# jedbrown/spectral-petsc

Measured on AMD Instinct MI355X. Metric: spectral matvecs/s and GB/s vs HBM roofline, 3D P^3 grid, higher is better.
Workload: dtype f64; 1 GPU; 3-D Poisson MatMult_Elliptic -dim 256,256,256 (gamma=0), global N(0,1) input seed 20240229; P=256, parallelism=single

## Files before the change

include/chebhip.h:

```cpp
#ifndef CHEBHIP_H
#define CHEBHIP_H

#ifdef __cplusplus
extern "C" {
#endif

enum {
  CHEBHIP_OK = 0,
  CHEBHIP_ERR_SIZE = 1,
  CHEBHIP_ERR_TDIM = 2,
  CHEBHIP_ERR_DIMS = 3,
  CHEBHIP_ERR_ARG = 4,
  CHEBHIP_ERR_DEVICE = 5,
  CHEBHIP_ERR_MEMORY = 6
};

const char *chebhip_last_error(void);
int chebhip_version(void);
const char *chebhip_arch(void);

typedef int (*chebhip_apply_fn)(void *ctx, const double *x_dev, double *y_dev, void *stream);
typedef int (*chebhip_reduce_fn)(void *ctx, double *vals_dev, int count, void *stream);

typedef struct cheb_plan cheb_plan;
// ... 41 lines not shown
int  cheb_modal_weights_host(int n, double *w);
int  cheb_modal_filter_matrix_host(int n, const double *sigma, double *F);

typedef struct cheb_points cheb_points;

int  cheb_points_create(int d, const int *dims, int nfields, cheb_points **out);
int  cheb_points_destroy(cheb_points *h);
long cheb_points_chunk(const cheb_points *h);
int  cheb_points_rows(cheb_points *h, int k, const double *x_dev, long m, double *R_dev, void *stream);
int  cheb_points_eval(cheb_points *h, const double *u_dev, const double *xi_dev, long npts, double *out_dev, void *stream);
enum { CHEB_SPREAD_ACCUMULATE = 1, CHEB_SPREAD_DELTA = 2 };
int  cheb_points_spread(cheb_points *h, const double *s_dev, const double *xi_dev, long npts, double *out_dev, int flags, void *stream);
long cheb_points_spread_pass(const cheb_points *h);
int  cheb_points_grid_reserve(cheb_points *h, const int *m_max);
int  cheb_points_eval_grid(cheb_points *h, const double *u_dev, const double *coords_dev, const int *m, double *out_dev, void *stream);
int  cheb_nodes_host(int n, double *x);
int  cheb_points_matrix_host(int n, int m, const double *x_host, double *R);
int  cheb_points_drows(cheb_points *h, int k, const double *x_dev, long m, double *R_dev, void *stream);
int  cheb_points_dmatrix_host(int n, int m, const double *x_host, double *R);
int  cheb_points_eval_deriv(cheb_points *h, const double *u_dev, const double *xi_dev, long npts, const int *deriv, double *out_dev,
                            void *stream);
int  cheb_points_spread_deriv(cheb_points *h, const double *s_dev, const double *xi_dev, long npts, const int *deriv, double *out_dev,
                              int flags, void *stream);
int  cheb_points_eval_grid_deriv(cheb_points *h, const double *u_dev, const double *coords_dev, const int *m, const int *deriv,
                                 double *out_dev, void *stream);
enum { CHEB_POINTS_GRAD_VALUE = 1 };
int  cheb_points_eval_grad(cheb_points *h, const double *u_dev, const double *xi_dev, long npts, const double *scale_host, int flags,
                           double *out_dev, void *stream);

typedef struct cheb_dealias cheb_dealias;

int  cheb_dealias_fine_size(int n);
int  cheb_dealias_matrix_host(int n, int m, int which, double *A);
int  cheb_dealias_create(int d, const int *dims, const int *dims_fine, int nfields, cheb_dealias **out);
int  cheb_dealias_destroy(cheb_dealias *h);
int  cheb_dealias_fine_dims(const cheb_dealias *h, int *dims_fine);
long cheb_dealias_size(const cheb_dealias *h);
long cheb_dealias_work_bytes(const cheb_dealias *h);
int  cheb_dealias_multiply(cheb_dealias *h, const double *u_dev, const double *v_dev, double *out_dev, void *stream);
int  cheb_dealias_reserve_advect(cheb_dealias *h);
int  cheb_dealias_advect(cheb_dealias *h, const double *vel_dev, const double *c_dev, double *out_dev, void *stream);

typedef struct cheb_reduce cheb_reduce;
enum { CHEB_W_INTEGRAL = 0, CHEB_W_MEAN = 1, CHEB_W_NODE = 2, CHEB_W_DNODE = 3, CHEB_W_POINT = 4, CHEB_W_DPOINT = 5 };

int  cheb_reduce_weights_host(int n, int kind, double arg, double *w);
int  cheb_reduce_create(int d, const int *dims, int nfields, const int *contract, cheb_reduce **out);
int  cheb_reduce_destroy(cheb_reduce *h);
int  cheb_reduce_set_weights(cheb_reduce *h, int k, const double *w_host);
long cheb_reduce_size(const cheb_reduce *h, int which);
int  cheb_reduce_slices(const cheb_reduce *h);
int  cheb_reduce_apply(cheb_reduce *h, const double *u_dev, const double *v_dev, double *out_dev, void *stream);

typedef struct cheb_stats cheb_stats;
enum { CHEB_STATS_UNIFORM = 0, CHEB_STATS_EDGES = 1 };

int  cheb_stats_spacing_host(int n, double *h);
int  cheb_stats_rate_host(int n, double s, double *r);
int  cheb_stats_check(int d, const int *dims, int nfields, int max_bins, int nbins);
int  cheb_stats_create(int d, const int *dims, int nfields, int max_bins, cheb_stats **out);
int  cheb_stats_destroy(cheb_stats *h);
int  cheb_stats_set_weights(cheb_stats *h, int k, const double *w_host);
long cheb_stats_size(const cheb_stats *h, int which);
int  cheb_stats_summary(cheb_stats *h, const double *u_dev, const double *center_dev, double *out_dev, void *stream);
int  cheb_stats_histogram(cheb_stats *h, const double *u_dev, const double *cond_dev, int mode, int nbins, const double *spec_dev,
                          double *out_dev, void *stream);
int  cheb_stats_cfl(cheb_stats *h, const double *vel_dev, const double *scale_host, double *out_dev, void *stream);

typedef struct cheb_grad cheb_grad;
enum { CHEB_INV_DIV = 1, CHEB_INV_VORT2 = 2, CHEB_INV_STRAIN2 = 4, CHEB_INV_GAMMA = 8, CHEB_INV_Q = 16, CHEB_INV_NORM2 = 32 };

int  cheb_grad_create(int d, const int *dims, const double *scale, cheb_grad **out);
int  cheb_grad_destroy(cheb_grad *h);
long cheb_grad_size(const cheb_grad *h);
long cheb_grad_work_size(const cheb_grad *h, int nfields);
int  cheb_grad_grad(cheb_grad *h, int nfields, const double *s_dev, double *out_dev, void *stream);
int  cheb_grad_tensor(cheb_grad *h, int nvec, const double *u_dev, double *G_dev, void *stream);
int  cheb_grad_div(cheb_grad *h, int nvec, const double *u_dev, double *out_dev, void *stream);
int  cheb_grad_curl(cheb_grad *h, int nvec, const double *u_dev, double *out_dev, void *stream);
int  cheb_grad_strain(cheb_grad *h, int nvec, const double *u_dev, double *out_dev, void *stream);
int  cheb_grad_laplacian(cheb_grad *h, int nfields, const double *s_dev, double *work_dev, double *out_dev, void *stream);
int  cheb_grad_invariants(cheb_grad *h, int nvec, const double *G_dev, unsigned mask, double *out_dev, void *stream);

typedef struct cheb_layout cheb_layout;
int  cheb_layout_create(int d, const int *dims, cheb_layout **out);
int  cheb_layout_destroy(cheb_layout *h);
long cheb_layout_size(const cheb_layout *h, int which);
int  cheb_layout_map_host(int d, const int *dims, int *map);
int  cheb_layout_unpack(cheb_layout *h, int ncomp, const double *xi_dev, long si, long oi, const double *xb_dev, long sb, long ob,
                        double *out_dev, void *stream);
int  cheb_layout_pack(cheb_layout *h, int ncomp, const double *fields_dev, double *xi_dev, long si, long oi, double *xb_dev, long sb, long ob,
                      void *stream);

typedef struct ell_op ell_op;

int ell_op_create(int d, const int *dims, ell_op **out);
int ell_op_destroy(ell_op *op);

long ell_op_local_size(const ell_op *op);
long ell_op_global_size(const ell_op *op);
long ell_op_dirichlet_size(const ell_op *op);

int ell_op_mult(ell_op *op, const double *U_dev, double *V_dev, void *stream);
int ell_op_mult_host(ell_op *op, const double *U_host, double *V_host);

int ell_op_function(ell_op *op, double gamma, double exponent, const double *U_dev,
                    const double *b_dev, double *rhs_dev, void *stream);
int ell_op_function_host(ell_op *op, double gamma, double exponent, const double *U_host,
                         const double *b_host, double *rhs_host);

int ell_op_set_dirichlet(ell_op *op, const double *values_host);

int ell_op_get_state(ell_op *op, int which, double *dst_host);
int ell_op_set_state(ell_op *op, int which, const double *src_host);

typedef int (*ell_dim0_fn)(void *ctx, int kind, int nfields, const double *in_dev, const double *acc_dev,
                           double alpha, double *out_dev, void *stream);
int ell_op_create_slab(int d, const int *dims, int lo, int hi, ell_dim0_fn dim0, void *dim0_ctx, ell_op **out);
int ell_op_pencil_sweep(ell_op *op, long ncol, const double *in_dev, double *out_dev, void *stream);

typedef struct stokes_op stokes_op;

int stokes_op_create(int d, const int *dims, stokes_op **out);
int stokes_op_destroy(stokes_op *op);
long stokes_op_size(const stokes_op *op, int which);

int stokes_op_set_rheology(stokes_op *op, int kind, double hardness, double exponent,
                           double regularization, double gamma0);
int stokes_op_set_dirichlet(stokes_op *op, const double *values_host);
int stokes_op_set_force(stokes_op *op, const double *force_host);

int stokes_op_mult(stokes_op *op, const double *xG_dev, double *yG_dev, void *stream);
int stokes_op_mult_vv(stokes_op *op, const double *vG_dev, double *vG_out_dev, void *stream);
int stokes_op_mult_pv(stokes_op *op, const double *vG_dev, double *pG_out_dev, void *stream);
int stokes_op_mult_vp(stokes_op *op, const double *pG_dev, double *vG_out_dev, void *stream);
int stokes_op_mult_schur(stokes_op *op, const double *pG_dev, double *pG_out_dev,
                         chebhip_apply_fn inner_solve, void *inner_ctx, void *stream);
int stokes_op_mult_vv_cm(stokes_op *op, const double *v_cm_dev, double *v_cm_out_dev, void *stream);
int stokes_op_mult_pv_cm(stokes_op *op, const double *v_cm_dev, double *pG_out_dev, void *stream);
int stokes_op_mult_vp_cm(stokes_op *op, const double *pG_dev, double *v_cm_out_dev, void *stream);
int stokes_op_mult_schur_cm(stokes_op *op, const double *pG_dev, double *pG_out_dev,
                            chebhip_apply_fn inner_solve_cm, void *inner_ctx, void *stream);
int stokes_op_set_inner_solver(stokes_op *op, int restart, double rtol, double atol, int max_it);
int stokes_op_inner_iterations(const stokes_op *op);
int stokes_op_set_inner_reduce(stokes_op *op, chebhip_reduce_fn reduce, void *ctx);
int stokes_op_function(stokes_op *op, const double *xG_dev, double *yG_dev, void *stream);
int stokes_op_get_state(stokes_op *op, int which, double *dst_host);
int stokes_op_set_state(stokes_op *op, int which, const double *src_host);

typedef int (*stokes_dim0_fn)(void *ctx, int kind, int nfields, const double *in_dev, const double *acc_dev,
                              double alpha, double *out_dev, void *stream);
int stokes_op_create_slab(int d, const int *dims, int lo, int hi, stokes_dim0_fn dim0, void *dim0_ctx, stokes_op **out);
int stokes_op_pencil_sweep(stokes_op *op, int nfields, long ncol, const double *in_dev, double *out_dev, void *stream);
int stokes_op_pencil_pressure(stokes_op *op, long ncol, double *p_pencil_dev, double *gp0_pencil_dev, void *stream);
int stokes_op_pencil_sweep_pressure(stokes_op *op, int nvel, long ncol, double *in_dev, double *out_dev, void *stream);

typedef struct chebhip_dist chebhip_dist;
typedef int (*chebhip_exchange_fn)(void *ctx, const double *send_dev, const long *send_counts, double *recv_dev,
                                   const long *recv_counts, void *stream);
int chebhip_dist_create(int d, const int *dims, int nranks, int rank, chebhip_dist **out);
int chebhip_dist_destroy(chebhip_dist *D);
long chebhip_dist_local_size(const chebhip_dist *D);
long chebhip_dist_slab_offset(const chebhip_dist *D);
int chebhip_dist_use_rccl(chebhip_dist *D, void *nccl_comm);
int chebhip_dist_set_exchange(chebhip_dist *D, chebhip_exchange_fn fn, void *ctx);
int chebhip_dist_mult(chebhip_dist *D, const double *U_slab_dev, double *V_slab_dev, void *stream);
int chebhip_dist_mult_batch(chebhip_dist *D, int nrhs, const double *U_slabs_dev, double *V_slabs_dev, void *stream);
int chebhip_rccl_unique_id(void *id128);
int chebhip_rccl_comm_create(int nranks, int rank, const void *id128, void **nccl_comm_out);
int chebhip_rccl_comm_destroy(void *nccl_comm);
int chebhip_rccl_reduce(void *nccl_comm, double *vals_dev, int count, void *stream);

typedef struct chebhip_comm chebhip_comm;
typedef struct chebhip_local_group chebhip_local_group;
typedef struct chebhip_ipc_group chebhip_ipc_group;
typedef int (*chebhip_exchangev_fn)(void *ctx, int nseg, const int *peers, const double *const *send_dev, const long *send_counts,
                                    double *const *recv_dev, const long *recv_counts, void *stream);
int chebhip_comm_create_rccl(void *nccl_comm, int nranks, int rank, chebhip_comm **out);
int chebhip_local_group_create(int nranks, chebhip_local_group **out);
int chebhip_local_group_destroy(chebhip_local_group *g);
int chebhip_local_group_abort(chebhip_local_group *g);
int chebhip_comm_create_local(chebhip_local_group *g, int rank, chebhip_comm **out);
int chebhip_comm_create_callback(int nranks, int rank, chebhip_exchangev_fn xfn, chebhip_reduce_fn rfn, void *ctx, chebhip_comm **out);
int chebhip_comm_create_null(int nranks, int rank, chebhip_comm **out);
int chebhip_comm_null_set_shadow(chebhip_comm *c, int k, const double *const *arrays);
int chebhip_ipc_group_open(const char *name, int nranks, int rank, chebhip_ipc_group **out);
int chebhip_ipc_group_close(chebhip_ipc_group *g);
int chebhip_ipc_group_abort(chebhip_ipc_group *g);
int chebhip_comm_create_ipc(chebhip_ipc_group *g, chebhip_comm *inner, chebhip_comm **out);
int chebhip_comm_destroy(chebhip_comm *c);
int chebhip_comm_size(const chebhip_comm *c);
int chebhip_comm_rank(const chebhip_comm *c);
int chebhip_comm_reduce(void *comm, double *vals_dev, int count, void *stream);
int chebhip_dist_use_comm(chebhip_dist *D, chebhip_comm *comm);

typedef struct chebhip_dist_stokes chebhip_dist_stokes;
typedef struct chebhip_fdpc chebhip_fdpc;
int chebhip_dist_stokes_create(int d, const int *dims, chebhip_comm *comm, chebhip_dist_stokes **out);
int chebhip_dist_stokes_destroy(chebhip_dist_stokes *D);
stokes_op *chebhip_dist_stokes_op(chebhip_dist_stokes *D);
int chebhip_dist_stokes_pc(chebhip_dist_stokes *D, chebhip_fdpc **out);
int chebhip_dist_stokes_ranges(const chebhip_dist_stokes *D, long *ranges4);
typedef struct chebhip_dist_ell chebhip_dist_ell;
int chebhip_dist_ell_create(int d, const int *dims, chebhip_comm *comm, chebhip_dist_ell **out);
int chebhip_dist_ell_destroy(chebhip_dist_ell *D);
ell_op *chebhip_dist_ell_op(chebhip_dist_ell *D);
int chebhip_dist_ell_pc(chebhip_dist_ell *D, chebhip_fdpc **out);
int chebhip_dist_ell_ranges(const chebhip_dist_ell *D, long *ranges4);

typedef struct chebhip_fgmres chebhip_fgmres;
int chebhip_fgmres_create(long n, int restart, chebhip_fgmres **out);
int chebhip_fgmres_set_reduce(chebhip_fgmres *k, chebhip_reduce_fn reduce, void *ctx);
int chebhip_fgmres_destroy(chebhip_fgmres *k);
int chebhip_fgmres_set_tolerances(chebhip_fgmres *k, double rtol, double atol, int max_it);
int chebhip_fgmres_solve(chebhip_fgmres *k, chebhip_apply_fn A, void *actx, chebhip_apply_fn M, void *mctx,
                         const double *b_dev, double *x_dev, int x_nonzero, void *stream);
int chebhip_fgmres_iterations(const chebhip_fgmres *k);
double chebhip_fgmres_residual(const chebhip_fgmres *k);
int chebhip_fgmres_reason(const chebhip_fgmres *k);

int ell_pc_create(ell_op *op, chebhip_fdpc **out);
int stokes_pc_create(stokes_op *op, chebhip_fdpc **out);
int chebhip_fdpc_destroy(chebhip_fdpc *pc);
typedef int (*chebhip_fdpc_dim0_fn)(void *ctx, int backward, int nfields, const double *in_dev, double *out_dev, void *stream);
int stokes_pc_create_slab(stokes_op *slab_op, long i0_offset, chebhip_fdpc_dim0_fn dim0, void *ctx, chebhip_fdpc **out);
int ell_pc_create_slab(ell_op *slab_op, long i0_offset, chebhip_fdpc_dim0_fn dim0, void *ctx, chebhip_fdpc **out);
int chebhip_fdpc_pencil_transform(chebhip_fdpc *pc, int backward, int nfields, long ncol, const double *in_dev, double *out_dev, void *stream);
int chebhip_fdpc_update(chebhip_fdpc *pc, void *stream);
int chebhip_fdpc_set_sweeps(chebhip_fdpc *pc, int sweeps);
int chebhip_fdpc_mult(chebhip_fdpc *pc, const double *x_dev, double *y_dev, void *stream);
int chebhip_fdpc_apply(void *pc, const double *r_dev, double *z_dev, void *stream);
int chebhip_fdpc_apply_cm(void *pc, const double *r_cm_dev, double *z_cm_dev, void *stream);
enum { CHEBHIP_FDPC_STEP_FORWARD = 0, CHEBHIP_FDPC_STEP_FORWARD_OVER_ETA = 1, CHEBHIP_FDPC_STEP_FORWARD_SCALED = 2,
       CHEBHIP_FDPC_STEP_ZSOLVE = 3, CHEBHIP_FDPC_STEP_SCALE = 4, CHEBHIP_FDPC_STEP_BACKWARD = 5 };
int chebhip_fdpc_step(chebhip_fdpc *pc, int k, int mode, const double *x_dev, double *y_dev, void *stream);
enum { CHEBHIP_FDPC_ROUTE_RAW = 1, CHEBHIP_FDPC_ROUTE_TWO_LAUNCH = 2, CHEBHIP_FDPC_ROUTE_GENERAL = 4, CHEBHIP_FDPC_ROUTE_FUSED_MUL = 8,
       CHEBHIP_FDPC_ROUTE_ETA_PASS = 16, CHEBHIP_FDPC_ROUTE_ZSOLVE = 32, CHEBHIP_FDPC_ROUTE_SCALE3 = 64, CHEBHIP_FDPC_ROUTE_SCALE_GENERAL = 128,
       CHEBHIP_FDPC_ROUTE_DENSE = 256 };
int chebhip_fdpc_step_route(chebhip_fdpc *pc, int k, int mode);
int chebhip_fdpc_line_host(int P, double *S, double *Sinv, double *lam);
int ell_pc_create_spectral(ell_op *op, double sigma, chebhip_fdpc **out);

typedef struct cheb_helmholtz cheb_helmholtz;
int  cheb_helmholtz_create(int d, const int *dims, double sigma, int nfields, cheb_helmholtz **out);
int  cheb_helmholtz_solve(cheb_helmholtz *h, const double *f_dev, double *u_dev, void *stream);
int  cheb_helmholtz_apply(void *h, const double *x_dev, double *y_dev, void *stream);
int  cheb_helmholtz_destroy(cheb_helmholtz *h);
long cheb_helmholtz_size(const cheb_helmholtz *h);
int  cheb_helmholtz_line_host(int P, double *S, double *Sinv, double *lam);
chebhip_fdpc *cheb_helmholtz_fdpc(cheb_helmholtz *h);

int  cheb_helmholtz_create_bc(int d, const int *dims, const double *bc, double sigma, int nfields, cheb_helmholtz **out);
int  cheb_helmholtz_solve_bc(cheb_helmholtz *h, const double *f_dev, const double *g_dev, double *u_dev, void *stream);
long cheb_helmholtz_full_size(const cheb_helmholtz *h);
long cheb_helmholtz_boundary_size(const cheb_helmholtz *h);
int  cheb_helmholtz_singular(const cheb_helmholtz *h);
int  cheb_helmholtz_line_bc_host(int P, const double *bc4, double *S, double *Sinv, double *lam,
                                 double *Q , double *L , double *Binv );
int  cheb_helmholtz_create_box(int d, const int *dims, const double *bc, const double *scale, double sigma, int nfields, cheb_helmholtz **out);
int  cheb_helmholtz_line_box_host(int P, const double *bc4, double s, double *S, double *Sinv, double *lam,
                                  double *Q , double *L , double *Binv );

typedef struct cheb_project cheb_project;
enum { CHEB_FACE_WALL = 0, CHEB_FACE_OPEN = 1 };
int  cheb_project_create(int d, const int *dims, const int *faces, const double *scale, int nvec, cheb_project **out);
int  cheb_project_destroy(cheb_project *h);
long cheb_project_size(const cheb_project *h, int which);
int  cheb_project_singular(const cheb_project *h);
int  cheb_project_faces_host(int d, const int *dims, int *face);
int  cheb_project_apply(cheb_project *h, const double *u_dev, const double *flux_dev, double *phi_dev, double *out_dev, void *stream);

typedef struct cheb_opfun cheb_opfun;
enum { CHEB_OPFUN_ONE = 0, CHEB_OPFUN_INV, CHEB_OPFUN_RES, CHEB_OPFUN_EXP, CHEB_OPFUN_PHI1, CHEB_OPFUN_PHI2, CHEB_OPFUN_PHI3, CHEB_OPFUN_POW };
typedef struct { int out, in, kind; double coef, tau, par; } cheb_opfun_term;
int  cheb_opfun_create(int d, const int *dims, const double *bc, const double *scale, double sigma, int nin, int nout, cheb_opfun **out);
int  cheb_opfun_destroy(cheb_opfun *h);
int  cheb_opfun_set_terms(cheb_opfun *h, int nterms, const cheb_opfun_term *terms);
int  cheb_opfun_check_terms(int nin, int nout, int nterms, const cheb_opfun_term *terms);
int  cheb_opfun_apply(cheb_opfun *h, const double *x_dev, double *y_dev, void *stream);
int  cheb_opfun_apply_full(cheb_opfun *h, const double *x_dev, double *yfull_dev, void *stream);
long cheb_opfun_size(const cheb_opfun *h, int which);
int  cheb_opfun_singular(const cheb_opfun *h);
int  cheb_opfun_weight_host(int kind, double tau, double par, double s, double *w);
int  cheb_opfun_weights_host(int kind, double tau, double par, long n, const double *s, double *w);
int  cheb_opfun_eval(int kind, double tau, double par, const double *s_dev, long n, double *w_dev, void *stream);

typedef struct stokes_saddle stokes_saddle;
int stokes_saddle_create(stokes_op *op, stokes_saddle **out);
int stokes_saddle_create_slab(stokes_op *slab_op, chebhip_fdpc *slab_pc, chebhip_reduce_fn reduce, void *reduce_ctx, stokes_saddle **out);
int stokes_saddle_destroy(stokes_saddle *s);
int stokes_saddle_set_type(stokes_saddle *s, int type);
int stokes_saddle_set_inner(stokes_saddle *s, int which, int max_it, double rtol);
int stokes_saddle_set_schur_jacobi(stokes_saddle *s, int on);
int stokes_saddle_set_pc_sweeps(stokes_saddle *s, int sweeps);
int stokes_saddle_setup(stokes_saddle *s, void *stream);
int stokes_saddle_apply(void *s, const double *x_dev, double *y_dev, void *stream);
int stokes_saddle_iterations(const stokes_saddle *s, int which);

int chebhip_set_option(const char *name, int value);
int chebhip_get_option(const char *name, int *value);
const char *chebhip_option_name(int index);

long chebhip_launch_count(void);

enum {
  CHEBHIP_STAGE_CHEB_APPLY = 0, CHEBHIP_STAGE_ELL_MULT, CHEBHIP_STAGE_ELL_FUNCTION, CHEBHIP_STAGE_STOKES_MULT,
  CHEBHIP_STAGE_STOKES_MULT_VV, CHEBHIP_STAGE_STOKES_MULT_PV, CHEBHIP_STAGE_STOKES_MULT_VP, CHEBHIP_STAGE_STOKES_FUNCTION,
  CHEBHIP_STAGE_STOKES_SCHUR, CHEBHIP_STAGE_FDPC_APPLY, CHEBHIP_STAGE_SADDLE_APPLY, CHEBHIP_STAGE_FGMRES_SOLVE,
  CHEBHIP_NSTAGES
};
int chebhip_timers_enable(int on);
int chebhip_timers_reset(void);
int chebhip_timers_read(int stage, double *total_ms, long *calls);
const char *chebhip_stage_name(int stage);

int stokes_op_viscosity_range(stokes_op *op, double *eta_min, double *eta_max, void *stream);
int stokes_op_write_vtk(stokes_op *op, const double *state_dev, const char *path);

#ifdef __cplusplus
}
#endif
#endif
```

spectral-petsc_amd/__init__.py:

```python
import ctypes as C
import os
import subprocess

_HERE = os.path.dirname(os.path.abspath(__file__))
LIB_PATH = os.environ.get("CHEBHIP_LIB_PATH") or os.path.join(_HERE, "libchebhip.so")
INCLUDE_DIR = os.path.join(os.path.dirname(_HERE), "include")

ABI_SYMBOLS = [
    "chebhip_last_error", "chebhip_version", "chebhip_arch", "chebhip_launch_count",
    "chebhip_set_option", "chebhip_get_option", "chebhip_option_name",
    "cheb_plan_create", "cheb_apply", "cheb_apply_host", "cheb_plan_destroy", "cheb_plan_size",
    "cheb_plan_create_trimmed", "cheb_apply_lap1d", "cheb_slab_pack", "cheb_slab_unpack_add",
    "ell_op_create", "ell_op_destroy", "ell_op_local_size", "ell_op_global_size",
    "ell_op_dirichlet_size", "ell_op_mult", "ell_op_mult_host", "ell_op_function",
    "ell_op_function_host", "ell_op_set_dirichlet", "ell_op_get_state", "ell_op_set_state",
    "ell_op_create_slab", "ell_op_pencil_sweep",
    "stokes_op_create", "stokes_op_destroy", "stokes_op_size", "stokes_op_set_rheology",
    "stokes_op_set_dirichlet", "stokes_op_set_force", "stokes_op_mult", "stokes_op_mult_vv",
    "stokes_op_mult_pv", "stokes_op_mult_vp", "stokes_op_mult_vv_cm", "stokes_op_mult_pv_cm", "stokes_op_mult_vp_cm", "stokes_op_mult_schur_cm", "stokes_op_function", "stokes_op_get_state",
    "stokes_op_set_state", "stokes_op_create_slab", "stokes_op_pencil_sweep", "stokes_op_pencil_pressure", "stokes_op_pencil_sweep_pressure", "stokes_op_mult_schur", "stokes_op_set_inner_solver", "stokes_op_inner_iterations", "stokes_op_set_inner_reduce",
    "chebhip_fgmres_create", "chebhip_fgmres_destroy", "chebhip_fgmres_set_tolerances", "chebhip_fgmres_solve",
    "chebhip_fgmres_iterations", "chebhip_fgmres_residual", "chebhip_fgmres_reason", "chebhip_fgmres_set_reduce",
    "ell_pc_create", "stokes_pc_create", "chebhip_fdpc_destroy", "chebhip_fdpc_update", "chebhip_fdpc_set_sweeps",
    "chebhip_fdpc_mult", "chebhip_fdpc_apply", "chebhip_fdpc_apply_cm",
    "chebhip_fdpc_step", "chebhip_fdpc_step_route", "chebhip_fdpc_line_host", "cheb_helmholtz_fdpc",
    "stokes_saddle_create", "stokes_saddle_destroy", "stokes_saddle_set_type", "stokes_saddle_set_inner",
    "stokes_saddle_setup", "stokes_saddle_apply", "stokes_saddle_iterations", "stokes_saddle_set_pc_sweeps", "stokes_saddle_set_schur_jacobi",
    "chebhip_timers_enable", "chebhip_timers_reset", "chebhip_timers_read", "chebhip_stage_name",
    "stokes_op_viscosity_range", "stokes_op_write_vtk",
    "chebhip_dist_create", "chebhip_dist_destroy", "chebhip_dist_local_size", "chebhip_dist_slab_offset",
    "chebhip_dist_use_rccl", "chebhip_dist_set_exchange", "chebhip_dist_mult", "chebhip_dist_mult_batch",
    "chebhip_rccl_unique_id", "chebhip_rccl_comm_create", "chebhip_rccl_comm_destroy", "chebhip_rccl_reduce",
    "chebhip_comm_create_rccl", "chebhip_local_group_create", "chebhip_local_group_destroy", "chebhip_local_group_abort",
    "chebhip_comm_create_local", "chebhip_comm_create_callback", "chebhip_comm_create_null", "chebhip_comm_null_set_shadow", "chebhip_comm_destroy", "chebhip_comm_size", "chebhip_comm_rank",
    "chebhip_ipc_group_open", "chebhip_ipc_group_close", "chebhip_ipc_group_abort", "chebhip_comm_create_ipc",
    "chebhip_comm_reduce", "chebhip_dist_use_comm",
    "chebhip_dist_stokes_create", "chebhip_dist_stokes_destroy", "chebhip_dist_stokes_op", "chebhip_dist_stokes_ranges",
    "chebhip_dist_ell_create", "chebhip_dist_ell_destroy", "chebhip_dist_ell_op", "chebhip_dist_ell_ranges",
    "stokes_pc_create_slab", "ell_pc_create_slab", "chebhip_fdpc_pencil_transform", "chebhip_dist_stokes_pc", "chebhip_dist_ell_pc",
    "stokes_saddle_create_slab",
    "cheb_resample_create", "cheb_resample_apply", "cheb_resample_destroy", "cheb_resample_size", "cheb_resample_matrix_host",
    "cheb_helmholtz_create", "cheb_helmholtz_solve", "cheb_helmholtz_apply", "cheb_helmholtz_destroy", "cheb_helmholtz_size",
    "cheb_helmholtz_line_host", "ell_pc_create_spectral",
    "cheb_helmholtz_create_bc", "cheb_helmholtz_solve_bc", "cheb_helmholtz_full_size", "cheb_helmholtz_boundary_size",
    "cheb_helmholtz_singular", "cheb_helmholtz_line_bc_host",
    "cheb_modal_create", "cheb_modal_destroy", "cheb_modal_size", "cheb_modal_spectrum_size", "cheb_modal_forward", "cheb_modal_backward",
    "cheb_modal_set_filter", "cheb_modal_filter", "cheb_modal_spectrum", "cheb_modal_integrate",
    "cheb_modal_matrix_host", "cheb_modal_weights_host", "cheb_modal_filter_matrix_host",
    "cheb_points_create", "cheb_points_destroy", "cheb_points_chunk", "cheb_points_rows", "cheb_points_eval",
    "cheb_points_spread", "cheb_points_spread_pass",
    "cheb_points_grid_reserve", "cheb_points_eval_grid", "cheb_nodes_host", "cheb_points_matrix_host",
    "cheb_points_drows", "cheb_points_dmatrix_host", "cheb_points_eval_deriv", "cheb_points_spread_deriv",
    "cheb_points_eval_grid_deriv", "cheb_points_eval_grad",
    "cheb_dealias_fine_size", "cheb_dealias_matrix_host", "cheb_dealias_create", "cheb_dealias_destroy", "cheb_dealias_fine_dims",
    "cheb_dealias_size", "cheb_dealias_work_bytes", "cheb_dealias_multiply", "cheb_dealias_reserve_advect", "cheb_dealias_advect",
    "cheb_reduce_weights_host", "cheb_reduce_create", "cheb_reduce_destroy", "cheb_reduce_set_weights", "cheb_reduce_size",
    "cheb_reduce_slices", "cheb_reduce_apply",
    "cheb_stats_spacing_host", "cheb_stats_rate_host", "cheb_stats_check", "cheb_stats_create", "cheb_stats_destroy",
    "cheb_stats_set_weights", "cheb_stats_size", "cheb_stats_summary", "cheb_stats_histogram", "cheb_stats_cfl",
    "cheb_grad_create", "cheb_grad_destroy", "cheb_grad_size", "cheb_grad_work_size", "cheb_grad_grad", "cheb_grad_tensor",
    "cheb_grad_div", "cheb_grad_curl", "cheb_grad_strain", "cheb_grad_laplacian", "cheb_grad_invariants",
    "cheb_layout_create", "cheb_layout_destroy", "cheb_layout_size", "cheb_layout_map_host", "cheb_layout_unpack", "cheb_layout_pack",
    "cheb_helmholtz_create_box", "cheb_helmholtz_line_box_host",
    "cheb_project_create", "cheb_project_destroy", "cheb_project_size", "cheb_project_singular", "cheb_project_faces_host",
    "cheb_project_apply",
    "cheb_opfun_create", "cheb_opfun_destroy", "cheb_opfun_set_terms", "cheb_opfun_apply", "cheb_opfun_apply_full", "cheb_opfun_size",
    "cheb_opfun_singular", "cheb_opfun_check_terms", "cheb_opfun_weight_host", "cheb_opfun_weights_host", "cheb_opfun_eval",
]


class OpFunTerm(C.Structure):
    _fields_ = [("out", C.c_int), ("inp", C.c_int), ("kind", C.c_int), ("coef", C.c_double), ("tau", C.c_double), ("par", C.c_double)]


class ChebhipError(RuntimeError):
    def __init__(self, code, msg):
        super().__init__("chebhip error %d: %s" % (code, msg))
        self.code = code


def build(force=False):
    src = os.path.join(_HERE, "csrc")
    if force:
        subprocess.check_call(["make", "-C", src, "-s", "clean"])
    subprocess.check_call(["make", "-C", src, "-s"])
    return LIB_PATH


_lib = None


def lib():
    global _lib
    if _lib is None:
        if not os.path.exists(LIB_PATH):
            raise ChebhipError(-1, "libchebhip.so not built (run __graft_entry__.build()); there is no CPU fallback")
        L = C.CDLL(LIB_PATH)
        dp, ip, vp = C.POINTER(C.c_double), C.POINTER(C.c_int), C.c_void_p
        L.chebhip_last_error.restype = C.c_char_p
        L.chebhip_arch.restype = C.c_char_p
        L.chebhip_launch_count.restype = C.c_long
        L.chebhip_set_option.argtypes = [C.c_char_p, C.c_int]
        L.chebhip_get_option.argtypes = [C.c_char_p, C.POINTER(C.c_int)]
        L.chebhip_option_name.argtypes = [C.c_int]
        L.chebhip_option_name.restype = C.c_char_p
        L.cheb_plan_create.argtypes = [C.c_int, C.c_int, ip, C.POINTER(vp)]
        L.cheb_apply.argtypes = [vp, vp, vp, vp]
        L.cheb_plan_create_trimmed.argtypes = [C.c_int, C.c_int, ip, C.POINTER(vp)]
        L.cheb_apply_lap1d.argtypes = [vp, vp, vp, C.c_double, vp, vp]
        lp = C.POINTER(C.c_long)
        L.cheb_slab_pack.argtypes = [C.c_long, C.c_long, C.c_long, C.c_int, lp, vp, vp, vp]
        L.cheb_slab_unpack_add.argtypes = [C.c_long, C.c_long, C.c_long, C.c_int, lp, vp, vp, C.c_double, vp, vp]
        L.cheb_apply_host.argtypes = [vp, dp, dp]
        L.cheb_plan_destroy.argtypes = [vp]
        L.cheb_plan_size.argtypes = [vp]
        L.cheb_plan_size.restype = C.c_long
        L.ell_op_create.argtypes = [C.c_int, ip, C.POINTER(vp)]
        L.ell_op_destroy.argtypes = [vp]
        L.ell_op_create_slab.argtypes = [C.c_int, ip, C.c_int, C.c_int, vp, vp, C.POINTER(vp)]
        L.ell_op_pencil_sweep.argtypes = [vp, C.c_long, vp, vp, vp]
        for f in (L.ell_op_local_size, L.ell_op_global_size, L.ell_op_dirichlet_size):
            f.argtypes = [vp]
            f.restype = C.c_long
        L.ell_op_mult.argtypes = [vp, vp, vp, vp]
        L.ell_op_mult_host.argtypes = [vp, dp, dp]
        L.ell_op_function.argtypes = [vp, C.c_double, C.c_double, vp, vp, vp, vp]
        L.ell_op_function_host.argtypes = [vp, C.c_double, C.c_double, dp, dp, dp]
        L.ell_op_set_dirichlet.argtypes = [vp, dp]
        L.ell_op_get_state.argtypes = [vp, C.c_int, dp]
        L.ell_op_set_state.argtypes = [vp, C.c_int, dp]
        L.stokes_op_create.argtypes = [C.c_int, ip, C.POINTER(vp)]
        L.stokes_op_destroy.argtypes = [vp]
        L.stokes_op_size.argtypes = [vp, C.c_int]
        L.stokes_op_size.restype = C.c_long
        L.stokes_op_set_rheology.argtypes = [vp, C.c_int, C.c_double, C.c_double, C.c_double, C.c_double]
        L.stokes_op_set_dirichlet.argtypes = [vp, dp]
        L.stokes_op_set_force.argtypes = [vp, dp]
        for f in (L.stokes_op_mult, L.stokes_op_mult_vv, L.stokes_op_mult_pv, L.stokes_op_mult_vp, L.stokes_op_function,
                  L.stokes_op_mult_vv_cm, L.stokes_op_mult_pv_cm, L.stokes_op_mult_vp_cm):
            f.argtypes = [vp, vp, vp, vp]
        L.stokes_op_mult_schur_cm.argtypes = [vp, vp, vp, vp, vp, vp]
        L.stokes_op_get_state.argtypes = [vp, C.c_int, dp]
        L.stokes_op_set_state.argtypes = [vp, C.c_int, dp]
        L.stokes_op_create_slab.argtypes = [C.c_int, ip, C.c_int, C.c_int, vp, vp, C.POINTER(vp)]
        L.stokes_op_pencil_sweep.argtypes = [vp, C.c_int, C.c_long, vp, vp, vp]
        L.stokes_op_pencil_pressure.argtypes = [vp, C.c_long, vp, vp, vp]
        L.stokes_op_mult_schur.argtypes = [vp, vp, vp, vp, vp, vp]
        L.stokes_op_set_inner_solver.argtypes = [vp, C.c_int, C.c_double, C.c_double, C.c_int]
        L.stokes_op_inner_iterations.argtypes = [vp]
        L.stokes_op_set_inner_reduce.argtypes = [vp, vp, vp]
        L.chebhip_fgmres_create.argtypes = [C.c_long, C.c_int, C.POINTER(vp)]
        L.chebhip_fgmres_destroy.argtypes = [vp]
        L.chebhip_fgmres_set_tolerances.argtypes = [vp, C.c_double, C.c_double, C.c_int]
        L.chebhip_fgmres_solve.argtypes = [vp, vp, vp, vp, vp, vp, vp, C.c_int, vp]
        L.chebhip_fgmres_iterations.argtypes = [vp]
        L.chebhip_fgmres_residual.argtypes = [vp]
        L.chebhip_fgmres_residual.restype = C.c_double
        L.chebhip_fgmres_reason.argtypes = [vp]
        L.chebhip_fgmres_set_reduce.argtypes = [vp, vp, vp]
        L.ell_pc_create.argtypes = [vp, C.POINTER(vp)]
        L.stokes_pc_create.argtypes = [vp, C.POINTER(vp)]
        L.chebhip_fdpc_destroy.argtypes = [vp]
        L.chebhip_fdpc_update.argtypes = [vp, vp]
        L.chebhip_fdpc_set_sweeps.argtypes = [vp, C.c_int]
        L.chebhip_fdpc_mult.argtypes = [vp, vp, vp, vp]
        L.chebhip_fdpc_apply.argtypes = [vp, vp, vp, vp]
        L.chebhip_fdpc_apply_cm.argtypes = [vp, vp, vp, vp]
        L.stokes_saddle_create.argtypes = [vp, C.POINTER(vp)]
        L.stokes_saddle_destroy.argtypes = [vp]
        L.stokes_saddle_set_type.argtypes = [vp, C.c_int]
        L.stokes_saddle_set_inner.argtypes = [vp, C.c_int, C.c_int, C.c_double]
        L.stokes_saddle_setup.argtypes = [vp, vp]
        L.stokes_saddle_apply.argtypes = [vp, vp, vp, vp]
        L.stokes_saddle_iterations.argtypes = [vp, C.c_int]
        L.stokes_saddle_set_pc_sweeps.argtypes = [vp, C.c_int]
        L.stokes_saddle_set_schur_jacobi.argtypes = [vp, C.c_int]
        L.chebhip_timers_enable.argtypes = [C.c_int]
        L.chebhip_timers_read.argtypes = [C.c_int, dp, C.POINTER(C.c_long)]
        L.chebhip_stage_name.argtypes = [C.c_int]
        L.chebhip_stage_name.restype = C.c_char_p
        L.stokes_op_viscosity_range.argtypes = [vp, dp, dp, vp]
        L.stokes_op_write_vtk.argtypes = [vp, vp, C.c_char_p]
        L.chebhip_dist_create.argtypes = [C.c_int, ip, C.c_int, C.c_int, C.POINTER(vp)]
        L.chebhip_dist_destroy.argtypes = [vp]
        for f in (L.chebhip_dist_local_size, L.chebhip_dist_slab_offset):
            f.argtypes = [vp]
            f.restype = C.c_long
        L.chebhip_dist_use_rccl.argtypes = [vp, vp]
        L.chebhip_dist_set_exchange.argtypes = [vp, vp, vp]
        L.chebhip_dist_mult.argtypes = [vp, vp, vp, vp]
        L.chebhip_dist_mult_batch.argtypes = [vp, C.c_int, vp, vp, vp]
        L.chebhip_rccl_unique_id.argtypes = [vp]
        L.chebhip_rccl_comm_create.argtypes = [C.c_int, C.c_int, vp, C.POINTER(vp)]
        L.chebhip_rccl_comm_destroy.argtypes = [vp]
        L.chebhip_rccl_reduce.argtypes = [vp, vp, C.c_int, vp]
        L.chebhip_comm_create_rccl.argtypes = [vp, C.c_int, C.c_int, C.POINTER(vp)]
        L.chebhip_local_group_create.argtypes = [C.c_int, C.POINTER(vp)]
        L.chebhip_local_group_destroy.argtypes = [vp]
        L.chebhip_local_group_abort.argtypes = [vp]
        L.chebhip_comm_create_local.argtypes = [vp, C.c_int, C.POINTER(vp)]
        L.chebhip_comm_create_callback.argtypes = [C.c_int, C.c_int, vp, vp, vp, C.POINTER(vp)]
        L.chebhip_comm_destroy.argtypes = [vp]
        L.chebhip_comm_create_null.argtypes = [C.c_int, C.c_int, C.POINTER(vp)]
        L.chebhip_comm_null_set_shadow.argtypes = [vp, C.c_int, C.POINTER(vp)]
        L.chebhip_ipc_group_open.argtypes = [C.c_char_p, C.c_int, C.c_int, C.POINTER(vp)]
        L.chebhip_ipc_group_close.argtypes = [vp]
        L.chebhip_ipc_group_abort.argtypes = [vp]
        L.chebhip_comm_create_ipc.argtypes = [vp, vp, C.POINTER(vp)]
        L.chebhip_comm_size.argtypes = [vp]
        L.chebhip_comm_rank.argtypes = [vp]
        L.chebhip_comm_reduce.argtypes = [vp, vp, C.c_int, vp]
        L.chebhip_dist_use_comm.argtypes = [vp, vp]
        for nm in ("stokes", "ell"):
            getattr(L, "chebhip_dist_%s_create" % nm).argtypes = [C.c_int, ip, vp, C.POINTER(vp)]
            getattr(L, "chebhip_dist_%s_destroy" % nm).argtypes = [vp]
            getattr(L, "chebhip_dist_%s_op" % nm).argtypes = [vp]
            getattr(L, "chebhip_dist_%s_op" % nm).restype = vp
            getattr(L, "chebhip_dist_%s_ranges" % nm).argtypes = [vp, lp]
            getattr(L, "chebhip_dist_%s_pc" % nm).argtypes = [vp, C.POINTER(vp)]
            getattr(L, "%s_pc_create_slab" % nm).argtypes = [vp, C.c_long, vp, vp, C.POINTER(vp)]
        L.chebhip_fdpc_pencil_transform.argtypes = [vp, C.c_int, C.c_int, C.c_long, vp, vp, vp]
        L.stokes_saddle_create_slab.argtypes = [vp, vp, vp, vp, C.POINTER(vp)]
        L.cheb_resample_create.argtypes = [C.c_int, ip, C.c_int, ip, C.c_int, C.c_int, C.POINTER(vp)]
        L.cheb_resample_apply.argtypes = [vp, vp, vp, vp]
        L.cheb_resample_destroy.argtypes = [vp]
        L.cheb_resample_size.argtypes = [vp, C.c_int]
        L.cheb_resample_size.restype = C.c_long
        L.cheb_resample_matrix_host.argtypes = [C.c_int, C.c_int, C.c_int, C.c_int, dp]
        L.cheb_helmholtz_create.argtypes = [C.c_int, ip, C.c_double, C.c_int, C.POINTER(vp)]
        for f in (L.cheb_helmholtz_solve, L.cheb_helmholtz_apply):
            f.argtypes = [vp, vp, vp, vp]
        L.cheb_helmholtz_destroy.argtypes = [vp]
        L.cheb_helmholtz_size.argtypes = [vp]
        L.cheb_helmholtz_size.restype = C.c_long
        L.cheb_helmholtz_line_host.argtypes = [C.c_int, dp, dp, dp]
        L.chebhip_fdpc_line_host.argtypes = [C.c_int, dp, dp, dp]
        L.chebhip_fdpc_step.argtypes = [vp, C.c_int, C.c_int, vp, vp, vp]
        L.chebhip_fdpc_step_route.argtypes = [vp, C.c_int, C.c_int]
        L.cheb_helmholtz_fdpc.argtypes = [vp]
        L.cheb_helmholtz_fdpc.restype = vp
        L.ell_pc_create_spectral.argtypes = [vp, C.c_double, C.POINTER(vp)]
        L.cheb_helmholtz_create_bc.argtypes = [C.c_int, ip, dp, C.c_double, C.c_int, C.POINTER(vp)]
        L.cheb_helmholtz_solve_bc.argtypes = [vp, vp, vp, vp, vp]
        for f in (L.cheb_helmholtz_full_size, L.cheb_helmholtz_boundary_size):
            f.argtypes = [vp]
            f.restype = C.c_long
        L.cheb_helmholtz_singular.argtypes = [vp]
        L.cheb_helmholtz_line_bc_host.argtypes = [C.c_int, dp, dp, dp, dp, dp, dp, dp]
        L.cheb_modal_create.argtypes = [C.c_int, ip, C.c_int, C.POINTER(vp)]
        L.cheb_modal_destroy.argtypes = [vp]
        for f in (L.cheb_modal_size, L.cheb_modal_spectrum_size):
            f.argtypes = [vp]
            f.restype = C.c_long
        for f in (L.cheb_modal_forward, L.cheb_modal_backward, L.cheb_modal_filter, L.cheb_modal_spectrum):
            f.argtypes = [vp, vp, vp, vp]
        L.cheb_modal_set_filter.argtypes = [vp, C.c_int, dp]
        L.cheb_modal_integrate.argtypes = [vp, vp, vp, vp, vp]
        L.cheb_modal_matrix_host.argtypes = [C.c_int, C.c_int, dp]
        L.cheb_modal_weights_host.argtypes = [C.c_int, dp]
        L.cheb_modal_filter_matrix_host.argtypes = [C.c_int, dp, dp]
        L.cheb_points_create.argtypes = [C.c_int, ip, C.c_int, C.POINTER(vp)]
        L.cheb_points_destroy.argtypes = [vp]
        L.cheb_points_chunk.argtypes = [vp]
        L.cheb_points_chunk.restype = C.c_long
        L.cheb_points_rows.argtypes = [vp, C.c_int, vp, C.c_long, vp, vp]
        L.cheb_points_eval.argtypes = [vp, vp, vp, C.c_long, vp, vp]
        L.cheb_points_spread.argtypes = [vp, vp, vp, C.c_long, vp, C.c_int, vp]
        L.cheb_points_spread_pass.argtypes = [vp]
        L.cheb_points_spread_pass.restype = C.c_long
        L.cheb_points_grid_reserve.argtypes = [vp, ip]
        L.cheb_points_eval_grid.argtypes = [vp, vp, vp, ip, vp, vp]
        L.cheb_nodes_host.argtypes = [C.c_int, dp]
        L.cheb_points_matrix_host.argtypes = [C.c_int, C.c_int, dp, dp]
        L.cheb_points_drows.argtypes = [vp, C.c_int, vp, C.c_long, vp, vp]
        L.cheb_points_dmatrix_host.argtypes = [C.c_int, C.c_int, dp, dp]
        L.cheb_points_eval_deriv.argtypes = [vp, vp, vp, C.c_long, ip, vp, vp]
        L.cheb_points_spread_deriv.argtypes = [vp, vp, vp, C.c_long, ip, vp, C.c_int, vp]
        L.cheb_points_eval_grid_deriv.argtypes = [vp, vp, vp, ip, ip, vp, vp]
        L.cheb_points_eval_grad.argtypes = [vp, vp, vp, C.c_long, dp, C.c_int, vp, vp]
        L.cheb_dealias_fine_size.argtypes = [C.c_int]
        L.cheb_dealias_matrix_host.argtypes = [C.c_int, C.c_int, C.c_int, dp]
        L.cheb_dealias_create.argtypes = [C.c_int, ip, ip, C.c_int, C.POINTER(vp)]
        L.cheb_dealias_destroy.argtypes = [vp]
        L.cheb_dealias_fine_dims.argtypes = [vp, ip]
        for f in (L.cheb_dealias_size, L.cheb_dealias_work_bytes):
            f.argtypes = [vp]
            f.restype = C.c_long
        L.cheb_dealias_reserve_advect.argtypes = [vp]
        for f in (L.cheb_dealias_multiply, L.cheb_dealias_advect):
            f.argtypes = [vp, vp, vp, vp, vp]
        L.cheb_reduce_weights_host.argtypes = [C.c_int, C.c_int, C.c_double, dp]
        L.cheb_reduce_create.argtypes = [C.c_int, ip, C.c_int, ip, C.POINTER(vp)]
        L.cheb_reduce_destroy.argtypes = [vp]
        L.cheb_reduce_set_weights.argtypes = [vp, C.c_int, dp]
        L.cheb_reduce_size.argtypes = [vp, C.c_int]
        L.cheb_reduce_size.restype = C.c_long
        L.cheb_reduce_slices.argtypes = [vp]
        L.cheb_reduce_apply.argtypes = [vp, vp, vp, vp, vp]
        L.cheb_stats_spacing_host.argtypes = [C.c_int, dp]
        L.cheb_stats_rate_host.argtypes = [C.c_int, C.c_double, dp]
        L.cheb_stats_check.argtypes = [C.c_int, ip, C.c_int, C.c_int, C.c_int]
        L.cheb_stats_create.argtypes = [C.c_int, ip, C.c_int, C.c_int, C.POINTER(vp)]
        L.cheb_stats_destroy.argtypes = [vp]
        L.cheb_stats_set_weights.argtypes = [vp, C.c_int, dp]
        L.cheb_stats_size.argtypes = [vp, C.c_int]
        L.cheb_stats_size.restype = C.c_long
        L.cheb_stats_summary.argtypes = [vp, vp, vp, vp, vp]
        L.cheb_stats_histogram.argtypes = [vp, vp, vp, C.c_int, C.c_int, vp, vp, vp]
        L.cheb_stats_cfl.argtypes = [vp, vp, dp, vp, vp]
        L.cheb_grad_create.argtypes = [C.c_int, ip, dp, C.POINTER(vp)]
        L.cheb_grad_destroy.argtypes = [vp]
        L.cheb_grad_size.argtypes = [vp]
        L.cheb_grad_size.restype = C.c_long
        L.cheb_grad_work_size.argtypes = [vp, C.c_int]
        L.cheb_grad_work_size.restype = C.c_long
        for f in (L.cheb_grad_grad, L.cheb_grad_tensor, L.cheb_grad_div, L.cheb_grad_curl, L.cheb_grad_strain):
            f.argtypes = [vp, C.c_int, vp, vp, vp]
        L.cheb_grad_laplacian.argtypes = [vp, C.c_int, vp, vp, vp, vp]
        L.cheb_grad_invariants.argtypes = [vp, C.c_int, vp, C.c_uint, vp, vp]
        L.cheb_layout_create.argtypes = [C.c_int, ip, C.POINTER(vp)]
        L.cheb_layout_destroy.argtypes = [vp]
        L.cheb_layout_size.argtypes = [vp, C.c_int]
        L.cheb_layout_size.restype = C.c_long
        L.cheb_layout_map_host.argtypes = [C.c_int, ip, ip]
        L.cheb_layout_unpack.argtypes = [vp, C.c_int, vp, C.c_long, C.c_long, vp, C.c_long, C.c_long, vp, vp]
        L.cheb_layout_pack.argtypes = [vp, C.c_int, vp, vp, C.c_long, C.c_long, vp, C.c_long, C.c_long, vp]
        L.cheb_helmholtz_create_box.argtypes = [C.c_int, ip, dp, dp, C.c_double, C.c_int, C.POINTER(vp)]
        L.cheb_helmholtz_line_box_host.argtypes = [C.c_int, dp, C.c_double, dp, dp, dp, dp, dp, dp]
        L.cheb_project_create.argtypes = [C.c_int, ip, ip, dp, C.c_int, C.POINTER(vp)]
        L.cheb_project_destroy.argtypes = [vp]
        L.cheb_project_size.argtypes = [vp, C.c_int]
        L.cheb_project_size.restype = C.c_long
        L.cheb_project_singular.argtypes = [vp]
        L.cheb_project_faces_host.argtypes = [C.c_int, ip, ip]
        L.cheb_project_apply.argtypes = [vp, vp, vp, vp, vp, vp]
        L.cheb_opfun_create.argtypes = [C.c_int, ip, dp, dp, C.c_double, C.c_int, C.c_int, C.POINTER(vp)]
        L.cheb_opfun_destroy.argtypes = [vp]
        L.cheb_opfun_set_terms.argtypes = [vp, C.c_int, C.POINTER(OpFunTerm)]
        L.cheb_opfun_check_terms.argtypes = [C.c_int, C.c_int, C.c_int, C.POINTER(OpFunTerm)]
        L.cheb_opfun_apply.argtypes = [vp, vp, vp, vp]
        L.cheb_opfun_apply_full.argtypes = [vp, vp, vp, vp]
        L.cheb_opfun_size.argtypes = [vp, C.c_int]
        L.cheb_opfun_size.restype = C.c_long
        L.cheb_opfun_singular.argtypes = [vp]
        L.cheb_opfun_weight_host.argtypes = [C.c_int, C.c_double, C.c_double, C.c_double, dp]
        L.cheb_opfun_weights_host.argtypes = [C.c_int, C.c_double, C.c_double, C.c_long, dp, dp]
        L.cheb_opfun_eval.argtypes = [C.c_int, C.c_double, C.c_double, vp, C.c_long, vp, vp]
        _lib = L
    return _lib


def set_option(name, value):
    _chk(lib().chebhip_set_option(name.encode(), int(value)))


def get_option(name):
    v = C.c_int()
    _chk(lib().chebhip_get_option(name.encode(), C.byref(v)))
    return v.value


def options():
    out, i = {}, 0
    while True:
        n = lib().chebhip_option_name(i).decode()
        if not n:
            return out
        out[n] = get_option(n)
        i += 1


def _chk(rc):
    if rc != 0:
        raise ChebhipError(rc, lib().chebhip_last_error().decode())


def _ints(v):
    return (C.c_int * len(v))(*[int(x) for x in v])


def _np_dp(a):
    import numpy as np
    assert isinstance(a, np.ndarray) and a.dtype == np.float64 and a.flags["C_CONTIGUOUS"]
    return a.ctypes.data_as(C.POINTER(C.c_double))


def _dev_ptr(t, n):
    import torch
    assert isinstance(t, torch.Tensor) and t.is_cuda and t.dtype == torch.float64 and t.is_contiguous()
    assert t.numel() == n, "expected %d elements, got %d" % (n, t.numel())
    return t.data_ptr()


def _stream():
    import torch
    return torch.cuda.current_stream().cuda_stream


def device_view(ptr, n):
    import torch

    if not ptr or int(n) == 0:
        return torch.empty(0, dtype=torch.float64, device=torch.device("cuda", torch.cuda.current_device()))

# ... 1467 lines not shown
```

spectral-petsc_amd/csrc/chebhip.hip:

```cpp
#include "../../include/chebhip.h"
#include "sweep.h"
#include "ops.h"
#include "timers.h"
#include <atomic>
#include <mutex>
#include <cmath>
#include <cstdarg>
#include <cstdio>
#include <cstdlib>
#include <cstring>
#include <map>
#include <new>
#include <string>
#include <vector>

using namespace chebhip;

static thread_local std::string g_err;
int chebhip_fail(int code, const char *fmt, ...) {
  char buf[512];
  va_list ap; va_start(ap, fmt); vsnprintf(buf, sizeof buf, fmt, ap); va_end(ap);
  g_err = buf;
  return code;
}

extern "C" const char *chebhip_last_error(void) { return g_err.c_str(); }
extern "C" int chebhip_version(void) { return 100; }
extern "C" const char *chebhip_arch(void) { return "gfx950"; }
extern "C" long chebhip_launch_count(void) { return sweep_launch_count(); }

extern "C" int chebhip_set_option(const char *name, int value) {
  if (!name) return chebhip_fail(CHEBHIP_ERR_ARG, "NULL option name");
  if (!strcmp(name, "no_rocblas")) { opt_set(OPT_VENDOR_GEMM, value ? 0 : 1); return 0; }
  const int id = opt_find(name);
  if (id < 0) return chebhip_fail(CHEBHIP_ERR_ARG, "unknown option '%s'", name);
  opt_set(id, value);
  return 0;
}
extern "C" int chebhip_get_option(const char *name, int *value) {
  if (!name || !value) return chebhip_fail(CHEBHIP_ERR_ARG, "NULL argument");
  if (!strcmp(name, "no_rocblas")) { *value = opt(OPT_VENDOR_GEMM) ? 0 : 1; return 0; }
  const int id = opt_find(name);
  if (id < 0) return chebhip_fail(CHEBHIP_ERR_ARG, "unknown option '%s'", name);
  *value = opt(id);
  return 0;
}
extern "C" const char *chebhip_option_name(int index) { return opt_name(index); }
static const double *g_stamp_buf = nullptr;
static int g_stamp_cnt = 0;
extern "C" void chebhip_debug_stamp_buffer(const void *dev) { g_stamp_buf = (const double *)dev; g_stamp_cnt = 0; }
const double *chebhip_stamp_buf() { return g_stamp_buf; }
int chebhip_stamp_next() { return g_stamp_cnt++; }

namespace {
struct Pending { int id; hipEvent_t e0, e1; };
std::mutex g_tm_mu;
bool g_tm_on = false;
std::vector<Pending> g_tm_pending;
double g_tm_ms[CHEBHIP_NSTAGES] = {0};
long g_tm_calls[CHEBHIP_NSTAGES] = {0};
const char *const g_tm_names[CHEBHIP_NSTAGES] = {
  "cheb_apply", "ell_op_mult", "ell_op_function", "stokes_op_mult", "stokes_op_mult_vv", "stokes_op_mult_pv", "stokes_op_mult_vp",
  "stokes_op_function", "stokes_op_mult_schur", "chebhip_fdpc_apply", "stokes_saddle_apply", "chebhip_fgmres_solve"};
void tm_drain_locked() {
  for (auto &p : g_tm_pending) {
    float ms = 0.f;
    if (hipEventSynchronize(p.e1) == hipSuccess && hipEventElapsedTime(&ms, p.e0, p.e1) == hipSuccess) { g_tm_ms[p.id] += ms; g_tm_calls[p.id]++; }
    (void)hipEventDestroy(p.e0); (void)hipEventDestroy(p.e1);
  }
  g_tm_pending.clear();
}
}
chebhip::StageTimer::StageTimer(int stage, void *stream) : id(stage), st((hipStream_t)stream), on(g_tm_on) {
  if (!on) return;
  if (hipEventCreate(&e0) != hipSuccess || hipEventRecord(e0, st) != hipSuccess) { on = false; if (e0) (void)hipEventDestroy(e0); }
}
chebhip::StageTimer::~StageTimer() {
  if (!on) return;
  hipEvent_t e1 = nullptr;
  if (hipEventCreate(&e1) != hipSuccess || hipEventRecord(e1, st) != hipSuccess) { (void)hipEventDestroy(e0); if (e1) (void)hipEventDestroy(e1); return; }
  std::lock_guard<std::mutex> lk(g_tm_mu);
  g_tm_pending.push_back({id, e0, e1});
  if (g_tm_pending.size() > 4096) tm_drain_locked();
}
extern "C" int chebhip_timers_enable(int on) { std::lock_guard<std::mutex> lk(g_tm_mu); g_tm_on = on != 0; return 0; }
extern "C" int chebhip_timers_reset(void) {
  std::lock_guard<std::mutex> lk(g_tm_mu);
  tm_drain_locked();
  for (int i = 0; i < CHEBHIP_NSTAGES; i++) { g_tm_ms[i] = 0.0; g_tm_calls[i] = 0; }
  return 0;
}
extern "C" int chebhip_timers_read(int stage, double *total_ms, long *calls) {
  if (stage < 0 || stage >= CHEBHIP_NSTAGES || !total_ms || !calls) return chebhip_fail(CHEBHIP_ERR_ARG, "stage %d out of range", stage);
  std::lock_guard<std::mutex> lk(g_tm_mu);
  tm_drain_locked();
  *total_ms = g_tm_ms[stage]; *calls = g_tm_calls[stage];
  return 0;
}
extern "C" const char *chebhip_stage_name(int stage) { return (stage >= 0 && stage < CHEBHIP_NSTAGES) ? g_tm_names[stage] : ""; }

struct cheb_plan {
  int rank = 0, tr = 0;
  std::vector<int> dims;
  long N = 0;
  unsigned inner = 1, ncols = 0;
  DiffMat mat;
  DiffMat lap;
  bool trimmed = false;
  double *hx = nullptr, *hy = nullptr;
};

static int check_geom(int rank, int tr, const int *dims, long *N, unsigned *inner, bool allow_long = false) {
  if (!dims || rank < 1 || rank > 16) return chebhip_fail(CHEBHIP_ERR_DIMS, "rank = %d must be in 1..16", rank);
  if (!(0 <= tr && tr < rank)) return chebhip_fail(CHEBHIP_ERR_TDIM, "tdim out of range");
  long n = 1, in = 1;
  for (int r = 0; r < rank; r++) {
    if (dims[r] < 1) return chebhip_fail(CHEBHIP_ERR_DIMS, "dims[%d] = %d must be >= 1", r, dims[r]);
    n *= dims[r];
    if (r > tr) in *= dims[r];
    if (n > 0x7fffffffL) return chebhip_fail(CHEBHIP_ERR_DIMS, "tensor of more than 2^31-1 points");
  }
  if (n < 2 || dims[tr] < 2) return chebhip_fail(CHEBHIP_ERR_SIZE, "n = %ld but must be >= 2", n);
  if (dims[tr] > 256 && !allow_long)
    return chebhip_fail(CHEBHIP_ERR_ARG, "dims[tr] = %d: the interior-layout (slab) plans support <= 256 points per line", dims[tr]);
  if (dims[tr] > 4096) return chebhip_fail(CHEBHIP_ERR_ARG, "dims[tr] = %d: at most 4096 points per line", dims[tr]);
  *N = n; *inner = (unsigned)in;
  return 0;
}

extern "C" int cheb_plan_create(int rank, int tr, const int *dims, cheb_plan **out) {
  if (!out) return chebhip_fail(CHEBHIP_ERR_ARG, "out is NULL");
  *out = nullptr;
  long N; unsigned inner;
  int rc = check_geom(rank, tr, dims, &N, &inner, true);
  if (rc) return rc;
  if ((rc = require_device())) return rc;
  cheb_plan *p = new (std::nothrow) cheb_plan;
  if (!p) return chebhip_fail(CHEBHIP_ERR_MEMORY, "out of host memory");
  p->rank = rank; p->tr = tr; p->dims.assign(dims, dims + rank);
  p->N = N; p->inner = inner; p->ncols = (unsigned)(N / dims[tr]);
  hipError_t e = hipSuccess;
  e = diffmat_create(dims[tr], &p->mat);
  if (e != hipSuccess) { delete p; return chebhip_fail(CHEBHIP_ERR_DEVICE, "plan matrices: %s", hipGetErrorString(e)); }
  *out = p;
  return 0;
}

extern "C" long cheb_plan_size(const cheb_plan *p) { return p ? p->N : -1; }

extern "C" int cheb_plan_create_trimmed(int rank, int tr, const int *dims, cheb_plan **out) {
  if (!out) return chebhip_fail(CHEBHIP_ERR_ARG, "out is NULL");
  *out = nullptr;
  if (!dims || rank < 1 || rank > 16) return chebhip_fail(CHEBHIP_ERR_DIMS, "rank = %d must be in 1..16", rank);
  if (!(0 <= tr && tr < rank)) return chebhip_fail(CHEBHIP_ERR_TDIM, "tdim out of range");
  std::vector<int> full(dims, dims + rank);
  if (dims[tr] < 1) return chebhip_fail(CHEBHIP_ERR_SIZE, "dims[tr] = %d stored points but must be >= 1", dims[tr]);
  full[tr] = dims[tr] + 2;
  long N; unsigned inner;
  int rc = check_geom(rank, tr, full.data(), &N, &inner);
  if (rc) return rc;
  if ((rc = require_device())) return rc;
  cheb_plan *p = new (std::nothrow) cheb_plan;
  if (!p) return chebhip_fail(CHEBHIP_ERR_MEMORY, "out of host memory");
  p->rank = rank; p->tr = tr; p->dims.assign(dims, dims + rank); p->trimmed = true;
  p->N = N / full[tr] * dims[tr]; p->inner = inner; p->ncols = (unsigned)(N / full[tr]);
  hipError_t e = diffmat_create(full[tr], &p->mat);
  if (e == hipSuccess) e = diffmat_create_lap(full[tr], &p->lap);
  if (e != hipSuccess) { diffmat_destroy(&p->mat); delete p; return chebhip_fail(CHEBHIP_ERR_DEVICE, "diffmat_create: %s", hipGetErrorString(e)); }
  *out = p;
  return 0;
}

extern "C" int cheb_apply_lap1d(cheb_plan *p, const double *x, const double *acc, double alpha,
                                double *y, void *stream) {
  if (!p || !x || !y) return chebhip_fail(CHEBHIP_ERR_ARG, "NULL argument");
  if (!p->trimmed) return chebhip_fail(CHEBHIP_ERR_ARG, "cheb_apply_lap1d needs a plan from cheb_plan_create_trimmed");
  if (x == y) return chebhip_fail(CHEBHIP_ERR_ARG, "x and y must be distinct");
  SweepParams sp = {};
  sp.ncols = p->ncols; sp.inner = p->inner;
  sp.in0 = x; sp.in_mode = IN_PLAIN;
  sp.alpha = alpha; sp.out = y;
  if (acc) { sp.out_mode = OUT_ACC; sp.acc = acc; } else sp.out_mode = OUT_STORE;
  HIP_TRY(sweep_launch(p->lap, sp, (hipStream_t)stream));
  return 0;
}

namespace chebhip {
int lap1d_gather_try(cheb_plan *p, const GatherSrc &g, double alpha, double *y, hipStream_t st, bool *done) {
  *done = false;
  if (!p || !p->trimmed || !y) return 0;
  SweepParams sp = {};
  sp.ncols = p->ncols; sp.inner = p->inner;
  sp.in_mode = IN_PLAIN; sp.alpha = alpha; sp.out = y; sp.out_mode = OUT_STORE;
  HIP_TRY(sweep_launch_gather(p->lap, sp, g, st, done));
  return 0;
}
}

namespace chebhip {
int lap1d_multi_gather_try(int n, cheb_plan *const *plans, const double *x, double *const *outs, cheb_plan *gp, const GatherSrc &g, double *gout,
                           double alpha, hipStream_t st, bool *done) {
  *done = false;
  if (n < 1 || n > 8 || !gp || !gp->trimmed || !gout) return 0;
  const DiffMat *m[9]; SweepParams sp[9];
  for (int k = 0; k < n; k++) {
    if (!plans[k] || !plans[k]->trimmed) return 0;
    sp[k] = SweepParams{};
    sp[k].ncols = plans[k]->ncols; sp[k].inner = plans[k]->inner;
    sp[k].in0 = x; sp[k].in_mode = IN_PLAIN; sp[k].alpha = alpha; sp[k].out = outs[k]; sp[k].out_mode = OUT_STORE;
    m[k] = &plans[k]->lap;
  }
  sp[n] = SweepParams{};
  sp[n].ncols = gp->ncols; sp[n].inner = gp->inner; sp[n].in_mode = IN_PLAIN; sp[n].alpha = alpha; sp[n].out = gout; sp[n].out_mode = OUT_STORE;
  m[n] = &gp->lap;
  HIP_TRY(sweep_launch_multi_gather_try(n + 1, m, sp, 1u << n, g, st, done));
  return 0;
}
}

namespace chebhip {
int lap1d_multi_try(int n, cheb_plan *const *plans, const double *x, double *const *outs, double alpha, hipStream_t st, bool *done) {
  *done = false;
  if (n < 2 || n > 9) return 0;
  const DiffMat *m[9]; SweepParams sp[9];
  for (int k = 0; k < n; k++) {
    if (!plans[k] || !plans[k]->trimmed) return 0;
    sp[k] = SweepParams{};
    sp[k].ncols = plans[k]->ncols; sp[k].inner = plans[k]->inner;
    sp[k].in0 = x; sp[k].in_mode = IN_PLAIN; sp[k].alpha = alpha; sp[k].out = outs[k]; sp[k].out_mode = OUT_STORE;
    m[k] = &plans[k]->lap;
  }
  HIP_TRY(sweep_launch_multi_try(n, m, sp, st, done));
  return 0;
}
}

extern "C" int cheb_apply(cheb_plan *p, const double *x, double *y, void *stream) {
  if (!p || !x || !y) return chebhip_fail(CHEBHIP_ERR_ARG, "NULL argument");
  if (x == y) return chebhip_fail(CHEBHIP_ERR_ARG, "x and y must be distinct (as every ChebMult call site)");
  if (p->trimmed) return chebhip_fail(CHEBHIP_ERR_ARG, "plan is trimmed: use cheb_apply_lap1d");
  StageTimer tm(CHEBHIP_STAGE_CHEB_APPLY, stream);
  SweepParams sp = {};
  sp.ncols = p->ncols; sp.inner = p->inner;
  sp.in0 = x; sp.out = y; sp.alpha = 1.0;
  sp.in_mode = IN_PLAIN; sp.out_mode = OUT_STORE;
  HIP_TRY(sweep_launch(p->mat, sp, (hipStream_t)stream));
  return 0;
}

extern "C" int cheb_apply_host(cheb_plan *p, const double *x, double *y) {
  if (!p || !x || !y) return chebhip_fail(CHEBHIP_ERR_ARG, "NULL argument");
  const size_t bytes = (size_t)p->N * sizeof(double);
  if (!p->hx) { HIP_TRY(hipMalloc((void **)&p->hx, bytes)); HIP_TRY(hipMalloc((void **)&p->hy, bytes)); }
  HIP_TRY(hipMemcpy(p->hx, x, bytes, hipMemcpyHostToDevice));
  int rc = cheb_apply(p, p->hx, p->hy, nullptr);
  if (rc) return rc;
  HIP_TRY(hipMemcpy(y, p->hy, bytes, hipMemcpyDeviceToHost));
  return 0;
}

extern "C" int cheb_plan_destroy(cheb_plan *p) {
  if (!p) return 0;
  diffmat_destroy(&p->mat);
  diffmat_destroy(&p->lap);
  if (p->hx) (void)hipFree(p->hx);
  if (p->hy) (void)hipFree(p->hy);
  delete p;
  return 0;
}

struct SlabSplit { int G; long c1[65]; };

__device__ __forceinline__ long slab_buf_index(const SlabSplit &sp, long m0, long M1, long R, long e) {
  const long i0 = e / (M1 * R), rem = e - i0 * (M1 * R);
  const long j = rem / R, r = rem - j * R;
  int s = 0;
  while (s + 1 < sp.G && j >= sp.c1[s + 1]) s++;
  const long w = sp.c1[s + 1] - sp.c1[s];
  return m0 * sp.c1[s] * R + (i0 * w + (j - sp.c1[s])) * R + r;
}

__global__ void k_slab_pack(SlabSplit sp, long m0, long M1, long R, const double *__restrict__ slab, double *__restrict__ buf) {
  const long n = m0 * M1 * R;
  for (long e = blockIdx.x * (long)blockDim.x + threadIdx.x; e < n; e += (long)gridDim.x * blockDim.x)
    buf[slab_buf_index(sp, m0, M1, R, e)] = slab[e];
}

__global__ void k_slab_unpack_add(SlabSplit sp, long m0, long M1, long R, const double *__restrict__ buf,
                                  const double *acc, double alpha, double *out) {
  const long n = m0 * M1 * R;
  for (long e = blockIdx.x * (long)blockDim.x + threadIdx.x; e < n; e += (long)gridDim.x * blockDim.x) {
    const double t = alpha * buf[slab_buf_index(sp, m0, M1, R, e)];
    out[e] = acc ? acc[e] + t : t;
  }
}

static int slab_split(int G, const long *c1, long M1, SlabSplit *sp) {
  if (G < 1 || G > 64 || !c1) return chebhip_fail(CHEBHIP_ERR_ARG, "G = %d must be in 1..64", G);
  sp->G = G;
  for (int s = 0; s <= G; s++) {
    sp->c1[s] = c1[s];
    if (c1[s] < 0 || c1[s] > M1 || (s > 0 && c1[s] < c1[s - 1])) return chebhip_fail(CHEBHIP_ERR_ARG, "column splits must be non-decreasing in 0..M1");
  }
  if (c1[0] != 0 || c1[G] != M1) return chebhip_fail(CHEBHIP_ERR_ARG, "column splits must cover 0..M1");
  return 0;
}

extern "C" int cheb_slab_pack(long m0, long M1, long R, int G, const long *c1, const double *slab, double *buf, void *stream) {
  if (!slab || !buf || m0 < 0 || M1 < 0 || R < 1) return chebhip_fail(CHEBHIP_ERR_ARG, "bad argument");
  SlabSplit sp; int rc = slab_split(G, c1, M1, &sp); if (rc) return rc;
  const long n = m0 * M1 * R;
  if (n == 0) return 0;
  long g = (n + 255) / 256; if (g > 4096) g = 4096;
  hipLaunchKernelGGL(k_slab_pack, dim3((unsigned)g), dim3(256), 0, (hipStream_t)stream, sp, m0, M1, R, slab, buf);
  HIP_TRY(hipGetLastError());
  return 0;
}

extern "C" int cheb_slab_unpack_add(long m0, long M1, long R, int G, const long *c1, const double *buf, const double *acc,
                                    double alpha, double *out, void *stream) {
  if (!buf || !out || m0 < 0 || M1 < 0 || R < 1) return chebhip_fail(CHEBHIP_ERR_ARG, "bad argument");
  SlabSplit sp; int rc = slab_split(G, c1, M1, &sp); if (rc) return rc;
  const long n = m0 * M1 * R;
  if (n == 0) return 0;
  long g = (n + 255) / 256; if (g > 4096) g = 4096;
  hipLaunchKernelGGL(k_slab_unpack_add, dim3((unsigned)g), dim3(256), 0, (hipStream_t)stream, sp, m0, M1, R, buf, acc, alpha, out);
  HIP_TRY(hipGetLastError());
  return 0;
}

__global__ void k_gather_bc(long N, const int *__restrict__ ixL, const double *__restrict__ U,
                            const double *__restrict__ dirloc, double *__restrict__ w0) {
// ... 808 lines not shown
```

spectral-petsc_amd/csrc/sweep.h:

```cpp
#pragma once
#include <hip/hip_runtime.h>
#include <vector>

namespace chebhip {

enum InMode : int {
  IN_PLAIN = 0,
  IN_GATHER = 1,
  IN_FLUX_ETA = 2,
  IN_FLUX_FULL = 3,
  IN_SUM3 = 4,
  IN_MUL = 5
};

enum OutMode : int {
  OUT_STORE = 0,
  OUT_ACC = 1,
  OUT_ACC_SCATTER = 2,
  OUT_ACC2 = 4,
  OUT_MUL = 3
};

enum CoefMode : int {
  COEF_UNIT = 0,
  COEF_ETA = 1,
  COEF_FULL = 2
};

struct SweepParams {
  int P;
  int H;
  unsigned ncols;
  unsigned inner;
  const double *in0, *in1, *in2, *in3, *in4;
  double *out;
  const double *acc;
  const double *acc2;
  const int *gcol;
  long gstride;
  double alpha;
  int in_mode, out_mode;
  const double *fragE, *fragO;
  const double *fragE2, *fragO2;
  const double *longDT;
  const double *longD;
  const double *zero;
  double *sink;
  unsigned ntiles;
  int sym;
  int raw;
  int trim;
  int coef_mode;
  double *gout;
  unsigned nouter, qmax;
  unsigned in_os, in_rs, acc_os, acc_rs, out_os, out_rs;
  unsigned in_bytes, acc_bytes, out_bytes;
  unsigned in_fblocks, in_fskip;
  unsigned in_fblocks_inv;
  unsigned gfield0;
};

struct DiffMat {
  int P = 0, H = 0;
  int KS = 0;
  int MTP = 0;
  double *fragE = nullptr, *fragO = nullptr;
  double *fragE2 = nullptr, *fragO2 = nullptr;
  double *longDT = nullptr;
  double *longD = nullptr;
  double *zero = nullptr;
  double *sink = nullptr;
  int sym = 0;
  int xl_ks = 0;
};

hipError_t diffmat_create(int P, DiffMat *out);
hipError_t diffmat_create_lap(int P, DiffMat *out);
hipError_t diffmat_create_pext(int P, DiffMat *out);
hipError_t diffmat_create_dd(int P, DiffMat *out);
void diffmat_destroy(DiffMat *m);
hipError_t diffmat_from_dense(int M, const long double *A, int sym, DiffMat *out);
hipError_t diffmat_from_blocks(int M, const long double *ME, const long double *MO, int sym, DiffMat *out);
void diffmat_dense_host(int P, double *D);
void resample_matrix_host(int n_in, int in_interior, int n_out, int out_interior, double *R);
void modal_matrix_host(int n, int which, double *M);
void modal_weights_host(int n, double *w);
void modal_filter_matrix_host(int n, const double *sigma, double *F);
int dealias_fine_size(int n);
void dealias_matrix_host(int n, int m, int which, double *A);
void points_nodes_host(int n, double *x);
void points_matrix_host(int n, int m, const double *x, double *R);
void points_dmatrix_host(int n, int m, const double *x, double *R);
enum { REDUCE_W_INTEGRAL = 0, REDUCE_W_MEAN, REDUCE_W_NODE, REDUCE_W_DNODE, REDUCE_W_POINT, REDUCE_W_DPOINT };
int reduce_weights_host(int n, int kind, double arg, double *w);
void stats_spacing_host(int n, double *h);
void stats_rate_host(int n, double s, double *r);

hipError_t sweep_launch(const DiffMat &m, SweepParams p, hipStream_t stream);

hipError_t fused_launch(const DiffMat &m, SweepParams p, hipStream_t stream);
void sweep_note_launch();

struct ResampleDir {
  const double *R;
  const double *x;
  double *y;
  unsigned O, K, M, Q, L;
};
hipError_t resample_launch(const ResampleDir &p, hipStream_t stream);
struct LineStep { int dir; const double *R; int m; };
hipError_t line_chain(int d, long *cur, long outer, long inner, int nsteps, const LineStep *steps, const double *src, double *dst,
                      double *const *work, hipStream_t stream);

struct F4Geom { unsigned os, ls, rs; };
struct Fused4Params {
  int P, H;
  unsigned nouter, qmax, ntiles, tpo, tpo_inv;
  const double *in; F4Geom gi; unsigned in_bytes;
  const void *coef; F4Geom gc; unsigned coef_bytes;
  double *gout; unsigned gout_bytes;
  const double *acc; F4Geom ga; unsigned acc_bytes;
  double *out; F4Geom go; unsigned out_bytes;
  const double *sub; unsigned sub_bytes;
  int trimf;
  double *w0out; unsigned w0_bytes;
  double alpha;
  int eta_square; double gamma4;
  const double *fragE2, *fragO2;
};
bool fused4_eligible(const DiffMat &m);
hipError_t fused4_launch(const DiffMat &m, Fused4Params p, bool jfast, bool full, bool acc, bool win, hipStream_t stream);

bool sweep_xl_eligible(const DiffMat &m, const SweepParams &p);
hipError_t sweep_xl_launch(const DiffMat &m, SweepParams p, hipStream_t stream);

bool sweep_vec_eligible(const DiffMat &m, const SweepParams &p);
bool sweep_takes_vec(const DiffMat &m, const SweepParams &p);
bool sweep_vec_raw_eligible(const DiffMat &m, const SweepParams &p);
hipError_t sweep_vec_launch(const DiffMat &m, SweepParams p, hipStream_t stream);
constexpr int GATHER_MAX = 16;
struct GatherSrc { const double *p[GATHER_MAX]; int s0[GATHER_MAX + 1]; unsigned lq[GATHER_MAX]; int pmax[GATHER_MAX]; int G; unsigned rowlen, col0;
                   double *dp[GATHER_MAX]; int push; };
hipError_t sweep_launch_gather(const DiffMat &m, SweepParams p, const GatherSrc &g, hipStream_t stream, bool *done);
hipError_t sweep_vec_launch_gather(const DiffMat &m, SweepParams p, const GatherSrc &g, hipStream_t stream, bool *done);
hipError_t sweep_vec_launch_multi(int n, const DiffMat *const *m, SweepParams *jobs, hipStream_t stream, bool *done);
hipError_t sweep_vec_launch_multi_gather(int n, const DiffMat *const *m, SweepParams *jobs, unsigned gmask, const GatherSrc &g, hipStream_t stream, bool *done);
hipError_t sweep_launch_multi_gather_try(int n, const DiffMat *const *m, const SweepParams *p, unsigned gmask, const GatherSrc &g, hipStream_t stream, bool *done);
hipError_t sweep_launch_multi(int n, const DiffMat *const *m, const SweepParams *p, hipStream_t stream);
hipError_t sweep_launch_multi_try(int n, const DiffMat *const *m, const SweepParams *p, hipStream_t stream, bool *done);

long sweep_launch_count();
}
struct cheb_plan;
struct stokes_op;
struct ell_op;
namespace chebhip {
bool ell_pencil_gather_supported(const ell_op *op);
int ell_pencil_gather_try(ell_op *op, long ncol, const GatherSrc &g, double *out, hipStream_t st, bool *done);
int stokes_pencil_gather_try(stokes_op *op, int kind, int nf, long ncol, const GatherSrc &g, double *out, hipStream_t st, bool *done);
bool stokes_pencil_gather_supported(const stokes_op *op);
int lap1d_multi_try(int n, cheb_plan *const *plans, const double *x, double *const *outs, double alpha, hipStream_t st, bool *done);
int lap1d_gather_try(cheb_plan *p, const GatherSrc &g, double alpha, double *y, hipStream_t st, bool *done);
int lap1d_multi_gather_try(int n, cheb_plan *const *plans, const double *x, double *const *outs, cheb_plan *gp, const GatherSrc &g, double *gout,
                           double alpha, hipStream_t st, bool *done);
int sweep_num_cus(hipError_t *err);

enum OptId { OPT_GENERAL_KERNELS = 0, OPT_SEPARATE_LAUNCHES, OPT_VENDOR_GEMM, OPT_NO_RAW_TRANSFORMS, OPT_EQUAL_SHARES, OPT_FORCE_GEMM,
             OPT_STOKES_SINGLE_STREAM, OPT_ETA_FROM_MEMORY, OPT_GATHER_PASS, OPT_RCCL_SELF_MESSAGES, OPT_LOCAL_TIMEOUT_S, OPT_FULL_STRESS, OPT_DIST_SINGLE_STREAM, OPT_LONG_LINES_GEMM, OPT_PRESSURE_PASSES, OPT_GENERAL_VISCOUS, OPT_POISSON_LAUNCHES, OPT_DIST_EXACT_ORDER, OPT_FDM_PASSES, OPT_SADDLE_NODE_MAJOR, OPT_STOKES_Z_SEPARATE, OPT_FDM_Z_SEPARATE, OPT_STOKES_PRESSURE_STREAM, OPT_KRYLOV_EXACT_NORM, OPT_STOKES_PRESSURE_SWEEPS, OPT_DIST_PACKED_EXCHANGE, OPT_POINTS_SPREAD_PASS, OPT_SWEEP_ALPHA_MULTIPLY, OPT_COUNT };
int opt(int id);
void opt_set(int id, int value);
const char *opt_name(int id);
int opt_find(const char *name);

bool fdm_line(int P, std::vector<long double> &S, std::vector<long double> &Sinv, std::vector<long double> &lam);
bool spec_line(int P, std::vector<long double> &S, std::vector<long double> &Sinv, std::vector<long double> &lam);
enum { SPEC_BC_SIZE = 1, SPEC_BC_COND, SPEC_BC_SINGULAR, SPEC_BC_EIG };
int spec_line_bc(int P, const double *bc4, std::vector<long double> &S, std::vector<long double> &Sinv, std::vector<long double> &lam,
                 std::vector<long double> &Q, std::vector<long double> &L, std::vector<long double> &Binv, bool &parity);
void centro_part(int M, const std::vector<long double> &A, int part, std::vector<long double> &out);

}
```

spectral-petsc_amd/csrc/sweep_vec.hip:

```cpp
#include "sweep.h"
#include "tile.h"
#include <cstdlib>
#include <type_traits>

const double *chebhip_stamp_buf();
int chebhip_stamp_next();

namespace chebhip {

template <bool ALIGNED16>
__device__ __forceinline__ void lds_put2(double *dst, double __attribute__((ext_vector_type(2))) v) {
  if (ALIGNED16) *(double __attribute__((ext_vector_type(2))) *)dst = v;
  else { dst[0] = v.x; dst[1] = v.y; }
}

template <int KS, bool JFAST, bool SUM3 = false, bool ACC = true>
__device__ __forceinline__ void vec1_body(const SweepParams &p, double *smem, const u32 BID, const u32 NBLK) {
  static_assert(KS <= 8, "lines of more than 64 points run vec4_body");
  static_assert(!SUM3 || !ACC, "IN_SUM3 exists for plain stores only");
  using G = TileGeom<KS, JFAST>;
  static_assert(G::CH >= 1 && (G::QSTEP % 2 == 0 || JFAST), "tile geometry");

#ifdef CHEB_STAMPS
  const unsigned long long st_entry = __builtin_amdgcn_s_memtime(), rt_entry = __builtin_amdgcn_s_memrealtime();
#endif
  const int tid = threadIdx.x, lane = tid & 63, w = tid >> 6;
  const int mt = w % G::MTP, ng = w / G::MTP;
  const int kq = lane >> 4, l16 = lane & 15;
  const int odd = l16 & 1, l16e = l16 & ~1;
  const int nn = p.P - 1, H = p.H;
  const u32 inner = p.inner, ncols = p.ncols;
  const u32 lineLen = (u32)p.P * inner;

  const u32 tpo = JFAST ? 1u : (inner + G::NT - 1) / G::NT;
  const u32 nxcd = (NBLK % 8 == 0) ? 8u : 1u;
  const u32 t_per = (p.ntiles + nxcd - 1) / nxcd;
  const u32 t_lo = (BID % nxcd) * t_per;
  const u32 t_hi = (t_lo + t_per < p.ntiles) ? t_lo + t_per : p.ntiles;
  const u32 t_step = NBLK / nxcd;
  u32 tile = t_lo + BID / nxcd;
  if (tile >= t_hi) return;

  const int ld_a = tid % G::LD_W, ld_b = tid / G::LD_W;
  const int ld_lds0 = JFAST ? ld_b * G::LDJ + 2 * ld_a : ld_b * G::NT + ((2 * ld_a) ^ ((ld_b & 1) << 4));

  constexpr bool TWO = !SUM3 && !ACC;
  struct Lines { d2 j[G::CH], m[G::CH]; };
  Lines LA, LB;
  const d2 *zero2 = (const d2 *)p.zero;

  const bool raw_in = p.raw == 2, raw_out = p.raw == 1;
  auto issue_loads = [&](u32 tl, bool valid, Lines &L) {
    d2 j1[SUM3 ? G::CH : 1], m1[SUM3 ? G::CH : 1], j2[SUM3 ? G::CH : 1], m2[SUM3 ? G::CH : 1];
    if (!JFAST) {
      const u32 o = tl / tpo, q0 = (tl - o * tpo) * G::NT;
      const u32 q = q0 + 2 * ld_a;
      const bool cv = valid && q < inner;
      const u32 base = o * lineLen + q;
      int jp = ld_b;
      u32 rel = (u32)jp * inner;
      const u32 top = base + (u32)nn * inner;
      asm volatile("" : "+v"(rel), "+v"(jp));
#pragma unroll
      for (int s = 0; s < G::CH; s++, jp += G::QSTEP, rel += G::QSTEP * inner) {
        const bool ok = cv && jp < H, okm = ok && nn - jp != jp;
        L.j[s] = *(ok ? (const d2 *)(p.in0 + (base + rel)) : zero2);
        L.m[s] = *(okm ? (const d2 *)(p.in0 + (top - rel)) : zero2);
        if (SUM3) {
          j1[s] = *(ok ? (const d2 *)(p.in1 + (base + rel)) : zero2); m1[s] = *(okm ? (const d2 *)(p.in1 + (top - rel)) : zero2);
          j2[s] = *(ok ? (const d2 *)(p.in2 + (base + rel)) : zero2); m2[s] = *(okm ? (const d2 *)(p.in2 + (top - rel)) : zero2);
        }
      }
    } else {
      const int j = 2 * ld_a;
#pragma unroll
      for (int s = 0; s < G::CH; s++) {
        const u32 c = tl * G::NT + ld_b + s * G::QSTEP;
        const bool ok = valid && c < ncols && j < H;
        const u32 base = (ok ? c : 0u) * lineLen;
        L.j[s] = *(ok ? (const d2 *)(p.in0 + (base + (u32)j)) : zero2);
        L.m[s] = *(ok ? (const d2 *)(p.in0 + (base + (u32)(nn - j - 1))) : zero2);
        if (SUM3) {
          j1[s] = *(ok ? (const d2 *)(p.in1 + (base + (u32)j)) : zero2); m1[s] = *(ok ? (const d2 *)(p.in1 + (base + (u32)(nn - j - 1))) : zero2);
          j2[s] = *(ok ? (const d2 *)(p.in2 + (base + (u32)j)) : zero2); m2[s] = *(ok ? (const d2 *)(p.in2 + (base + (u32)(nn - j - 1))) : zero2);
        }
      }
    }
    if (SUM3) {
#pragma unroll
      for (int s = 0; s < G::CH; s++) { L.j[s] = (L.j[s] + j1[s]) + j2[s]; L.m[s] = (L.m[s] + m1[s]) + m2[s]; }
    }
  };

  auto park_chunk = [&](int buf, const Lines &L) {
    double *dE = smem + buf * (2 * G::LDS_ELEMS), *dO = dE + G::LDS_ELEMS;
#pragma unroll
    for (int s = 0; s < G::CH; s++) {
      const int idx = ld_lds0 + s * G::LDS_QSTEP;
      const d2 rj = L.j[s], rm = L.m[s];
      d2 e, o;
      if (!JFAST) {
        const bool mid = 2 * (ld_b + s * G::QSTEP) == nn;
        if (raw_in) { e = rj; o = rm; }
        else { e = rj + rm; o = rj - rm; }
        if (mid) o = d2{0.0, 0.0};
      } else {
        const bool v1 = 2 * ld_a + 1 < H;
        if (raw_in) { e = d2{rj.x, v1 ? rj.y : 0.0}; o = d2{rm.y, v1 ? rm.x : 0.0}; }
        else {
          e = d2{rj.x + rm.y, v1 ? rj.y + rm.x : 0.0};
          o = d2{rj.x - rm.y, v1 ? rj.y - rm.x : 0.0};
        }
      }
      lds_put2<!JFAST || (G::LDJ % 2 == 0)>(dE + idx, e);
      lds_put2<!JFAST || (G::LDJ % 2 == 0)>(dO + idx, o);
    }
  };

  double ae[KS], ao[KS];
  if (!SUM3) issue_loads(tile, true, LA);
  if (TWO) issue_loads(tile + t_step, tile + t_step < t_hi, LB);
#pragma unroll
  for (int s = 0; s < KS; s++) {
    ae[s] = p.fragE[((long)(mt * KS + s)) * 64 + lane];
    ao[s] = p.fragO[((long)(mt * KS + s)) * 64 + lane];
  }
  if (SUM3) issue_loads(tile, true, LA);
  __builtin_amdgcn_s_waitcnt(0x0F70);

  const int i0 = mt * 16 + (JFAST ? l16 : kq);
  const bool mul_on = ACC && (p.out_mode == OUT_MUL);
  const bool acc2_on = ACC && (p.out_mode == OUT_ACC2);
  const bool acc_on = ACC && ((p.out_mode == OUT_ACC) || mul_on || acc2_on);
  const double alpha = p.alpha;

#ifdef CHEB_STAMPS
  unsigned long long st_pre = 0, st_chain = 0, st_post = 0, st_bar = 0, st_t0, st_t1, st_begin, st_loop, st_end, st_tiles = 0;
#define STAMP(v) do { __builtin_amdgcn_sched_barrier(0); v = __builtin_amdgcn_s_memtime(); __builtin_amdgcn_s_waitcnt(0xC07F); __builtin_amdgcn_sched_barrier(0); } while (0)
#else
#define STAMP(v) do { } while (0)
#endif
#ifdef CHEB_STAMPS
  STAMP(st_begin);
#endif
  park_chunk(0, LA);
  if (!TWO && tile + t_step < t_hi) issue_loads(tile + t_step, true, LA);
  lds_barrier();
#ifdef CHEB_STAMPS
  STAMP(st_loop);
#endif

  auto tile_body = [&](int cur, auto &&issue_fn, auto &&park_fn) {
    const double *sE = smem + cur * (2 * G::LDS_ELEMS), *sO = sE + G::LDS_ELEMS;
    const u32 t_o = tile / tpo, t_q0 = (tile - t_o * tpo) * G::NT;
#ifdef CHEB_STAMPS
    STAMP(st_t0); st_tiles++;
#endif
    issue_fn();
    const int nb = ng * 16;

    u32 a_hi[2], a_lo[2];
    bool ok_hi[2], ok_lo[2], fold[2];
    d2 acc_hi[2], acc_lo[2];
#pragma unroll
    for (int rp = 0; rp < 2; rp++) {
      const int r = 2 * rp + odd;
      if (!JFAST) {
        const u32 q = t_q0 + nb + l16e;
        const int i = i0 + 4 * r;
        const u32 b = t_o * lineLen + q;
        ok_hi[rp] = q < inner && i < H;
        ok_lo[rp] = ok_hi[rp] && (nn - i != i);
        fold[rp] = false;
        a_hi[rp] = b + (u32)i * inner;
        a_lo[rp] = b + (u32)(nn - i) * inner;
      } else {
        const u32 c = tile * G::NT + nb + 4 * r + kq;
        const int ie = mt * 16 + l16e;
        const u32 b = (c < ncols ? c : 0u) * lineLen;
        ok_hi[rp] = c < ncols && ie < H;
        fold[rp] = ok_hi[rp] && (ie + 1 >= H);
        ok_lo[rp] = ok_hi[rp] && !fold[rp];
        a_hi[rp] = b + (u32)ie;
        a_lo[rp] = b + (u32)(nn - ie - 1);
      }
      acc_hi[rp] = d2{0.0, 0.0}; acc_lo[rp] = d2{0.0, 0.0};
    }
    if (acc_on) {
#pragma unroll
      for (int rp = 0; rp < 2; rp++) {
        acc_hi[rp] = *(ok_hi[rp] ? (const d2 *)(p.acc + a_hi[rp]) : zero2);
        acc_lo[rp] = *(ok_lo[rp] ? (const d2 *)(p.acc + a_lo[rp]) : zero2);
        if (acc2_on) {
          acc_hi[rp] = acc_hi[rp] + *(ok_hi[rp] ? (const d2 *)(p.acc2 + a_hi[rp]) : zero2);
          acc_lo[rp] = acc_lo[rp] + *(ok_lo[rp] ? (const d2 *)(p.acc2 + a_lo[rp]) : zero2);
        }
      }
    }

#ifdef CHEB_STAMPS
    STAMP(st_t1); st_pre += st_t1 - st_t0;
#endif
    v4d ce = {0.0, 0.0, 0.0, 0.0}, co = {0.0, 0.0, 0.0, 0.0};
    {
      const int frag = G::frag(nb, l16, kq);
      const double *fE = sE + frag, *fO = sO + frag;
      double fb[2][4];
      fb[0][0] = fE[0]; fb[0][1] = fE[G::KSTR]; fb[0][2] = fO[0]; fb[0][3] = fO[G::KSTR];
#pragma unroll
      for (int g = 0; g < KS / 2; g++) {
        const int cb = g & 1, nbuf = cb ^ 1;
        if (g + 1 < KS / 2) {
          fb[nbuf][0] = fE[(2 * g + 2) * G::KSTR]; fb[nbuf][1] = fE[(2 * g + 3) * G::KSTR];
          fb[nbuf][2] = fO[(2 * g + 2) * G::KSTR]; fb[nbuf][3] = fO[(2 * g + 3) * G::KSTR];
        }
        __builtin_amdgcn_sched_barrier(0);
        if (!JFAST) {
          ce = __builtin_amdgcn_mfma_f64_16x16x4f64(ae[2 * g], fb[cb][0], ce, 0, 0, 0);
          co = __builtin_amdgcn_mfma_f64_16x16x4f64(ao[2 * g], fb[cb][2], co, 0, 0, 0);
          ce = __builtin_amdgcn_mfma_f64_16x16x4f64(ae[2 * g + 1], fb[cb][1], ce, 0, 0, 0);
          co = __builtin_amdgcn_mfma_f64_16x16x4f64(ao[2 * g + 1], fb[cb][3], co, 0, 0, 0);
        } else {
          ce = __builtin_amdgcn_mfma_f64_16x16x4f64(fb[cb][0], ae[2 * g], ce, 0, 0, 0);
          co = __builtin_amdgcn_mfma_f64_16x16x4f64(fb[cb][2], ao[2 * g], co, 0, 0, 0);
          ce = __builtin_amdgcn_mfma_f64_16x16x4f64(fb[cb][1], ae[2 * g + 1], ce, 0, 0, 0);
          co = __builtin_amdgcn_mfma_f64_16x16x4f64(fb[cb][3], ao[2 * g + 1], co, 0, 0, 0);
        }
      }
    }
#ifdef CHEB_STAMPS
    STAMP(st_t0); st_chain += st_t0 - st_t1;
#endif
    park_fn();

    double hi[4], lo[4];
#pragma unroll
    for (int r = 0; r < 4; r++) {
      if (raw_out) { hi[r] = ce[r]; lo[r] = co[r]; }
      else { hi[r] = ce[r] + co[r]; lo[r] = p.sym ? ce[r] - co[r] : co[r] - ce[r]; }
    }
#pragma unroll
    for (int rp = 0; rp < 2; rp++) {
      const double own_hi = odd ? hi[2 * rp + 1] : hi[2 * rp], snd_hi = odd ? hi[2 * rp] : hi[2 * rp + 1];
      const double own_lo = odd ? lo[2 * rp + 1] : lo[2 * rp], snd_lo = odd ? lo[2 * rp] : lo[2 * rp + 1];
      const double rcv_hi = swap1(snd_hi), rcv_lo = swap1(snd_lo);
      d2 vh = odd ? d2{rcv_hi, own_hi} : d2{own_hi, rcv_hi};
      d2 vl;
      if (!JFAST) vl = odd ? d2{rcv_lo, own_lo} : d2{own_lo, rcv_lo};
      else vl = odd ? d2{own_lo, rcv_lo} : d2{rcv_lo, own_lo};
      if (JFAST && fold[rp]) vh = d2{vh.x, odd ? rcv_lo : own_lo};
      if (!ACC) { vh = alpha * vh; vl = alpha * vl; }
      else if (mul_on) { vh = acc_hi[rp] * (alpha * vh); vl = acc_lo[rp] * (alpha * vl); }
      else { vh = acc_hi[rp] + alpha * vh; vl = acc_lo[rp] + alpha * vl; }
      if (ok_hi[rp]) *(d2 *)(p.out + a_hi[rp]) = vh;
      if (ok_lo[rp]) *(d2 *)(p.out + a_lo[rp]) = vl;
    }
#ifdef CHEB_STAMPS
    STAMP(st_t1); st_post += st_t1 - st_t0;
#endif
    lds_barrier();
#ifdef CHEB_STAMPS
    STAMP(st_t0); st_bar += st_t0 - st_t1;
#endif
  };

  const u32 t2 = 2 * t_step;
  if (!TWO) {
    for (int cur = 0; tile < t_hi; tile += t_step, cur ^= 1)
      tile_body(cur, [] {}, [&] {
        if (tile + t_step < t_hi) park_chunk(cur ^ 1, LA);
        if (tile + t2 < t_hi) issue_loads(tile + t2, true, LA);
      });
  } else {
    for (;;) {
      tile_body(0, [&] { issue_loads(tile + t2, tile + t2 < t_hi, LA); }, [&] { park_chunk(1, LB); });
      tile += t_step; if (tile >= t_hi) break;
      tile_body(1, [&] { issue_loads(tile + t2, tile + t2 < t_hi, LB); }, [&] { park_chunk(0, LA); });
      tile += t_step; if (tile >= t_hi) break;
    }
  }
#ifdef CHEB_STAMPS
  STAMP(st_end);
  if (lane == 0 && p.in4) {
    unsigned long long *dbg = (unsigned long long *)p.in4 + ((size_t)BID * 8 + w) * 16;
    dbg[0] = st_pre; dbg[1] = st_chain; dbg[2] = st_post; dbg[3] = st_bar;
    dbg[4] = st_loop - st_begin; dbg[5] = st_end - st_loop; dbg[6] = st_begin; dbg[7] = st_end;
    dbg[8] = st_begin - st_entry; dbg[10] = __builtin_amdgcn_s_memrealtime() - rt_entry; dbg[11] = st_end - st_entry;
    dbg[9] = st_tiles;
  }
#endif
}

template <int KS, bool JFAST, bool ACC>
__global__ __launch_bounds__(512, 4) void cheb_sweep_vec_kernel(const SweepParams p) {
  __shared__ double smem[TileGeom<KS, JFAST>::LDS_DOUBLES];
  vec1_body<KS, JFAST, false, ACC>(p, smem, blockIdx.x, gridDim.x);
}

#ifdef CHEB_STAMPS
#define STAMP3(k_) do { unsigned long long t_; __builtin_amdgcn_sched_barrier(0); \
    asm volatile("s_memtime %0\n\ts_waitcnt lgkmcnt(0)" : "=s"(t_) :: "memory"); __builtin_amdgcn_sched_barrier(0); \
    st_seg[k_] += t_ - st_prev; st_prev = t_; } while (0)
#define STAMP3_MARK(v_) do { unsigned long long t_; __builtin_amdgcn_sched_barrier(0); \
    asm volatile("s_memtime %0\n\ts_waitcnt lgkmcnt(0)" : "=s"(t_) :: "memory"); __builtin_amdgcn_sched_barrier(0); v_ = t_; st_prev = t_; } while (0)
#else
#define STAMP3(k_) do { } while (0)
#define STAMP3_MARK(v_) do { } while (0)
#endif

constexpr int V4_FRAG_AHEAD = 2;

template <int KS, bool JFAST, int MODE, int RAW = 0, int INM = 0, int GATH = 0, int SG = 0>
__device__ __forceinline__ void vec4_body(const SweepParams &p, double *smem, const u32 BID, const u32 NBLK, const GatherSrc *gs = nullptr) {
  static_assert(!GATH || (!JFAST && MODE == 0 && RAW == 0 && INM == 0), "the gather loader exists for strided lines, plain input, STORE");
  constexpr bool PUSH = GATH == 2;
  constexpr bool ACC = MODE != 0, MUL = MODE == 2, ACC2 = MODE == 3;
  static_assert(!ACC2 || RAW == 0, "OUT_ACC2 has no raw mode");
  constexpr bool ONEBUF = ACC2 && KS == 32;
  static_assert(INM == 0 || (RAW == 1 && MODE == 0), "IN_MUL exists for the raw forward transform with a plain store only");
  static_assert(RAW == 0 || MODE != 1, "the raw modes (sweep.h) are STORE / MUL only");
  static_assert(!MUL || RAW == 1, "OUT_MUL exists for the raw forward transform only");
  static_assert(SG == 0 || (MODE == 0 && RAW == 0 && INM == 0 && GATH == 0), "the sign-only store exists for the plain STORE launch");
  using G = TileGeom<KS, JFAST>;
  constexpr u32 INVALID = 0x80000000u, T_INVALID = 0x40000000u;
  static_assert(KS >= 16 && G::CH >= 1, "v4 needs two sub-tiles per tile");

#ifdef CHEB_STAMPS
  unsigned long long st_seg[5] = {0, 0, 0, 0, 0}, st_prev = 0, st_begin = 0, st_loop = 0, st_first = 0;
  const unsigned long long rt_begin = __builtin_amdgcn_s_memrealtime();
#endif
  const int tid = threadIdx.x, lane = tid & 63, w = tid >> 6;
  STAMP3_MARK(st_begin);
  const int mt = w % G::MTP, ng = w / G::MTP;
  const int kq = lane >> 4, l16 = lane & 15;
  const bool odd = l16 & 1; const int l16e = l16 & ~1;
  const int nn = p.P - 1, H = p.H;
  const u32 qmax = p.qmax;

  const __amdgpu_buffer_rsrc_t r_in = __builtin_amdgcn_make_buffer_rsrc((void *)p.in0, 0, p.in_bytes, 0x00020000);
  const __amdgpu_buffer_rsrc_t r_in1 = __builtin_amdgcn_make_buffer_rsrc((void *)(INM ? p.in1 : p.in0), 0, INM ? p.in_bytes : 0u, 0x00020000);
  const __amdgpu_buffer_rsrc_t r_acc = __builtin_amdgcn_make_buffer_rsrc((void *)(ACC ? p.acc : p.in0), 0, ACC ? p.acc_bytes : 0u, 0x00020000);
  const __amdgpu_buffer_rsrc_t r_acc2 = __builtin_amdgcn_make_buffer_rsrc((void *)(ACC2 ? p.acc2 : p.in0), 0, ACC2 ? p.acc_bytes : 0u, 0x00020000);
  const __amdgpu_buffer_rsrc_t r_out = __builtin_amdgcn_make_buffer_rsrc((void *)p.out, 0, p.out_bytes, 0x00020000);

  double ae[KS], ao[G::KR > 0 ? G::KR : 1];
  double *aoL = smem + 4 * G::LDS_ELEMS + (w * G::NFL) * 64 + lane;

  const u32 tpo = JFAST ? 1u : (qmax + G::NT - 1) / G::NT;
  const TileWalk wk = tile_walk(BID, NBLK, p.ntiles);
  const u32 t_hi = wk.t_hi, t_step = wk.t_step;

  const int ld_a = tid % G::LD_W, ld_b = tid / G::LD_W;
  const int ld_lds0 = JFAST ? ld_b * G::LDJ + 2 * ld_a : ld_b * G::NT + ((2 * ld_a) ^ ((ld_b & 1) << 4));
  const u32 in_os8 = p.in_os * 8u, in_rs8 = p.in_rs * 8u;
  const u32 lj = JFAST ? (u32)ld_b * in_os8 + (u32)(2 * ld_a) * 8u : (u32)(2 * ld_a) * 8u + (u32)ld_b * in_rs8;
  const u32 lm = JFAST ? (u32)ld_b * in_os8 + (u32)(nn - 2 * ld_a - 1) * 8u : (u32)(2 * ld_a) * 8u + (u32)(nn - ld_b) * in_rs8;
  const u32 slot8 = JFAST ? (u32)G::QSTEP * in_os8 : (u32)G::QSTEP * in_rs8;
  auto tile_off = [&](u32 tl, bool valid, u32 os8) -> u32 {
    if (JFAST) return valid ? tl * G::NT * os8 : T_INVALID;
    const u32 o = tl / tpo, q0 = (tl - o * tpo) * G::NT;
    return valid ? o * os8 + q0 * 8u : T_INVALID;
  };

  const u32 fb = p.in_fblocks, fskip8 = p.in_fskip * 8u;
  auto in_tile_off = [&](u32 tl) -> u32 {
    u32 off = tile_off(tl, true, in_os8);
    if (fb) off += __umulhi(JFAST ? tl * G::NT : tl / tpo, p.in_fblocks_inv) * fskip8;
    return off;
  };

  typedef const d2 __attribute__((address_space(1))) *gd2p;
  unsigned long long gb_j[GATH ? G::ITEMS : 1], gb_m[GATH ? G::ITEMS : 1];
  u32 glq_j[GATH ? G::ITEMS : 1], glq_m[GATH ? G::ITEMS : 1];
  unsigned long long pb_hi[2] = {0, 0}, pb_lo[2] = {0, 0}, psink = 0;
  u32 pl_hi[2] = {0, 0}, pl_lo[2] = {0, 0};
  if constexpr (GATH) {
    unsigned long long *gRB = (unsigned long long *)(smem + 2 * G::LDS_ELEMS);
    u32 *gRL = (u32 *)(gRB + 2 * G::HP);
    unsigned long long *gDB = (unsigned long long *)(gRL + 2 * G::HP);
    if (tid <= nn) {
      const int gG = gs->G;
      unsigned long long pb = (unsigned long long)gs->p[0], db = PUSH ? (unsigned long long)gs->dp[0] : 0ull; u32 lq = gs->lq[0]; int s0v = gs->s0[0], pmv = gs->pmax[0];
#pragma unroll
      for (int k = 1; k < GATHER_MAX; k++) {
        const bool c = (k < gG) && (tid >= gs->s0[k]);
        pb = c ? (unsigned long long)gs->p[k] : pb; lq = c ? gs->lq[k] : lq; s0v = c ? gs->s0[k] : s0v; pmv = c ? gs->pmax[k] : pmv;
        if constexpr (PUSH) db = c ? (unsigned long long)gs->dp[k] : db;
      }
      int pl = tid - s0v; if (pl > pmv - 1) pl = pmv - 1; if (pl < 0) pl = 0;
      const unsigned long long ro = ((unsigned long long)pl * gs->rowlen + gs->col0) * 8ull;
      gRB[tid] = pb + ro;
      gRL[tid] = lq;
      if constexpr (PUSH) gDB[tid] = db + ro;
    }
    __syncthreads();
    if constexpr (PUSH) {
#pragma unroll
      for (int rp = 0; rp < 2; rp++) {
        int i = mt * 16 + kq + 4 * (2 * rp + (odd ? 1 : 0)); if (i > nn) i = nn;
        pb_hi[rp] = gDB[i]; pl_hi[rp] = gRL[i];
        pb_lo[rp] = gDB[nn - i]; pl_lo[rp] = gRL[nn - i];
      }
      psink = (unsigned long long)p.out + (unsigned long long)tid * 16ull;
    }
#pragma unroll
    for (int sg = 0; sg < G::ITEMS; sg++) {
      int row = ld_b + sg * G::QSTEP; if (row > nn) row = nn;
      gb_j[sg] = gRB[row]; glq_j[sg] = gRL[row];
      gb_m[sg] = gRB[nn - row]; glq_m[sg] = gRL[nn - row];
    }
  }
  d2 rjA[G::CH], rmA[G::CH], rjB[G::CH], rmB[G::CH];
  constexpr int ECH = INM ? G::CH : 1;
  d2 ejA[ECH], emA[ECH], ejB[ECH], emB[ECH];
  d2 accX_hi[2], accX_lo[2], accY_hi[2], accY_lo[2];
  d2 acc2X_hi[2], acc2X_lo[2], acc2Y_hi[2], acc2Y_lo[2];

  auto issue_loads = [&](u32 tl, bool valid, int chunk, d2 (&rj)[G::CH], d2 (&rm)[G::CH]) {
    if constexpr (GATH) {
      const u32 tle = valid ? tl : 0u;
      const u32 gf0 = p.gfield0;
      const u32 o = tle / tpo, q0 = (tle - o * tpo) * G::NT;
      u32 qq = q0 + 2u * (u32)ld_a; if (qq > qmax - 2u) qq = qmax - 2u;
#pragma unroll
      for (int s = 0; s < G::CH; s++) {
        const int sg = chunk * G::CH + s;
        rj[s] = *(gd2p)(gb_j[sg] + ((unsigned long long)(o + gf0) * glq_j[sg] + qq) * 8ull);
        rm[s] = *(gd2p)(gb_m[sg] + ((unsigned long long)(o + gf0) * glq_m[sg] + qq) * 8ull);
      }
      return;
    }
    const u32 t0 = in_tile_off(tl);
    if constexpr (INM != 0) {
      d2 (&ej)[ECH] = (&rj == &rjA) ? ejA : ejB; d2 (&em)[ECH] = (&rj == &rjA) ? emA : emB;
#pragma unroll
      for (int s = 0; s < G::CH; s++) {
        const u32 so = (u32)(chunk * G::CH + s) * slot8;
        ej[s] = ld16(r_in1, lj + (valid ? t0 + so : T_INVALID));
        em[s] = ld16(r_in1, lm + (valid ? (JFAST ? t0 + so : t0 - so) : T_INVALID));
      }
    }
#pragma unroll
    for (int s = 0; s < G::CH; s++) {
      const u32 so = (u32)(chunk * G::CH + s) * slot8;
      rj[s] = ld16(r_in, lj + (valid ? t0 + so : T_INVALID));
      rm[s] = ld16(r_in, lm + (valid ? (JFAST ? t0 + so : t0 - so) : T_INVALID));
    }
  };
  const bool oddP = (p.P & 1) != 0;
  auto park_chunk = [&](int buf, int chunk, const d2 (&rj)[G::CH], const d2 (&rm)[G::CH]) {
    double *dE = smem + buf * (2 * G::LDS_ELEMS), *dO = dE + G::LDS_ELEMS;
#pragma unroll
    for (int s = 0; s < G::CH; s++) {
      const int idx = ld_lds0 + (chunk * G::CH + s) * G::LDS_QSTEP;
      d2 e, o;
      d2 xj = rj[s], xm = rm[s];
      if constexpr (INM != 0) {
        const d2 (&ej)[ECH] = (&rj == &rjA) ? ejA : ejB; const d2 (&em)[ECH] = (&rj == &rjA) ? emA : emB;
        xj = xj * ej[s]; xm = xm * em[s];
      }
      if (RAW == 2) {
        e = xj;
        o = JFAST ? d2{xm.y, xm.x} : xm;
      } else if (!JFAST) {
        e = xj + xm;
        o = xj - xm;
        if (oddP) { asm volatile("" ::: "memory"); const bool mid = 2 * (ld_b + (chunk * G::CH + s) * G::QSTEP) == nn; if (mid) e = xj; }
      } else {
        e = d2{xj.x + xm.y, xj.y + xm.x};
        o = d2{xj.x - xm.y, xj.y - xm.x};
      }
      lds_put2<!JFAST || (G::LDJ % 2 == 0)>(dE + idx, e);
      lds_put2<!JFAST || (G::LDJ % 2 == 0)>(dO + idx, o);
    }
  };

  const int i0 = mt * 16 + (JFAST ? l16 : kq);
  u32 o_hi[2], o_lo[2], c_hi[2], c_lo[2];
  bool fold[2] = {false, false};
#pragma unroll
  for (int rp = 0; rp < 2; rp++) {
    const int r = 2 * rp + (odd ? 1 : 0);
    if (!JFAST) {
      const int i = i0 + 4 * r;
      const bool ok = i < H, okl = ok & (nn - i != i);
      o_hi[rp] = ok ? (u32)l16e * 8u + (u32)i * (p.out_rs * 8u) : INVALID;
      o_lo[rp] = okl ? (u32)l16e * 8u + (u32)(nn - i) * (p.out_rs * 8u) : INVALID;
      c_hi[rp] = (u32)l16e * 8u + (u32)(ok ? i : 0) * (p.acc_rs * 8u);
      c_lo[rp] = (u32)l16e * 8u + (u32)(ok ? nn - i : 0) * (p.acc_rs * 8u);
    } else {
      const int ie = mt * 16 + l16e;
      const bool ok = ie < H;
      fold[rp] = ok & (ie + 1 >= H);
      const bool okl = ok & !fold[rp];
      o_hi[rp] = ok ? (u32)(4 * r + kq) * (p.out_os * 8u) + (u32)ie * 8u : INVALID;
      o_lo[rp] = okl ? (u32)(4 * r + kq) * (p.out_os * 8u) + (u32)(nn - ie - 1) * 8u : INVALID;
      c_hi[rp] = (u32)(4 * r + kq) * (p.acc_os * 8u) + (u32)(ok ? ie : 0) * 8u;
      c_lo[rp] = (u32)(4 * r + kq) * (p.acc_os * 8u) + (u32)(ok ? nn - ie - 1 : 0) * 8u;
    }
  }
  const u32 out_os8 = p.out_os * 8u, acc_os8 = p.acc_os * 8u;
  const u32 sub8_out = JFAST ? 16u * out_os8 : 16u * 8u, sub8_acc = JFAST ? 16u * acc_os8 : 16u * 8u;
  const u32 ng8_out = (u32)ng * G::NSUB * sub8_out, ng8_acc = (u32)ng * G::NSUB * sub8_acc;
  const double alpha = p.alpha, alpha_lo = (p.sym || RAW == 1) ? p.alpha : -p.alpha;

  auto acc_issue = [&](u32 tl, bool valid, int sub, d2 (&ah)[2], d2 (&al)[2]) {
    if (!ACC) return;
    const u32 t0 = tile_off(tl, valid, acc_os8) + ng8_acc + (u32)sub * sub8_acc;
#pragma unroll
    for (int rp = 0; rp < 2; rp++) { ah[rp] = ld16(r_acc, c_hi[rp] + t0); al[rp] = ld16(r_acc, c_lo[rp] + t0); }
    if constexpr (ACC2) {
      d2 (&bh)[2] = (&ah == &accX_hi) ? acc2X_hi : acc2Y_hi; d2 (&bl)[2] = (&ah == &accX_hi) ? acc2X_lo : acc2Y_lo;
#pragma unroll
      for (int rp = 0; rp < 2; rp++) { bh[rp] = ld16(r_acc2, c_hi[rp] + t0); bl[rp] = ld16(r_acc2, c_lo[rp] + t0); }
    }
  };

  u32 tile = wk.first();
  if (tile >= t_hi) return;
  issue_loads(tile, true, 0, rjA, rmA); issue_loads(tile, true, 1, rjB, rmB);
  constexpr int FA = (V4_FRAG_AHEAD < KS / 2) ? V4_FRAG_AHEAD : KS / 2;
  auto frag_pair = [&](int g) {
    const d2 ve = ((const d2 *)p.fragE2)[((long)(mt * (KS / 2) + g)) * 64 + lane];
    ae[2 * g] = ve.x; ae[2 * g + 1] = ve.y;
    if (2 * g + 1 < G::KR) {
      const d2 vo = ((const d2 *)p.fragO2)[((long)(mt * (KS / 2) + g)) * 64 + lane];
      ao[2 * g] = vo.x; ao[2 * g + 1] = vo.y;
    }
  };
  constexpr int GL = G::KR / 2;
  constexpr int NTL = (G::NFL > 0) ? KS / 2 - GL : 1;
  d2 tl[NTL];
  if constexpr (G::NFL > 0) {
#pragma unroll
    for (int g = GL; g < KS / 2; g++) tl[g - GL] = ((const d2 *)p.fragO2)[((long)(mt * (KS / 2) + g)) * 64 + lane];
  }
#pragma unroll
  for (int g = 0; g < FA; g++) frag_pair(g);
  if constexpr (G::NFL > 0) {
#pragma unroll
    for (int g = GL; g < KS / 2; g++) {
      if (2 * g >= G::KR) aoL[(2 * g - G::KR) * 64] = tl[g - GL].x; else ao[2 * g] = tl[g - GL].x;
      if (2 * g + 1 >= G::KR) aoL[(2 * g + 1 - G::KR) * 64] = tl[g - GL].y; else ao[2 * g + 1] = tl[g - GL].y;
    }
  }
#ifdef CHEB_STAMPS
  unsigned long long st_wait = 0, st_park = 0;
  STAMP3_MARK(st_wait);
#endif
  park_chunk(0, 0, rjA, rmA); park_chunk(0, 1, rjB, rmB);
#ifdef CHEB_STAMPS
  STAMP3_MARK(st_park);
#endif

  auto chain = [&](const double *sE, const double *sO, int sub, int g_issue, int g_park, v4d &ce, v4d &co, auto &&issue_fn, auto &&park_fn, auto &&grp_fn) {
    const int nb = (ng * G::NSUB + sub) * 16;
    ce = v4d{0.0, 0.0, 0.0, 0.0}; co = v4d{0.0, 0.0, 0.0, 0.0};
    const int frag = G::frag(nb, l16, kq);
    mfma_chain<KS, JFAST, G::KSTR>(sE + frag, sO + frag, ce, co, [&](int k) { return ae[k]; }, [&](int k) { return frag_odd<G::KR>(k, ao, aoL); },
                                   [&](int g) { grp_fn(g); if (g == g_issue) issue_fn(); if (g == g_park) park_fn(); });
  };
  auto epilogue = [&](u32 tl, int sub, const v4d &ce, const v4d &co, const d2 (&acc_hi)[2], const d2 (&acc_lo)[2]) {
    u32 t0 = tile_off(tl, true, out_os8) + ng8_out + (u32)sub * sub8_out;
    u32 t0v = t0;
    if (!JFAST) {
      const u32 o = tl / tpo, q = (tl - o * tpo) * G::NT + (ng * G::NSUB + sub) * 16 + l16e;
      t0v = (q < qmax) ? t0 : T_INVALID;
    }
    double hi[4], lo[4];
#pragma unroll
    for (int r = 0; r < 4; r++) {
      if (RAW == 1) { hi[r] = ce[r]; lo[r] = co[r]; }
      else if (SG) { hi[r] = -ce[r] - co[r]; lo[r] = co[r] - ce[r]; }
      else { hi[r] = ce[r] + co[r]; lo[r] = ce[r] - co[r]; }
    }
#pragma unroll
    for (int rp = 0; rp < 2; rp++) {
      const double ha = hi[2 * rp], hb = hi[2 * rp + 1], la = lo[2 * rp], lb = lo[2 * rp + 1];
      d2 vh, vl;
      if (RAW == 1) {
        const double hbe = bc_even(hb), hao = bc_odd(ha), lbe = bc_even(lb), lao = bc_odd(la);
        vh = d2{odd ? hbe : ha, odd ? hb : hao};
        if (!JFAST) vl = d2{odd ? lbe : la, odd ? lb : lao};
        else vl = d2{odd ? lb : lao, odd ? lbe : la};
      } else {
        double hx, hy, lx, ly;
        xpair(ha, hb, hx, hy); xpair(la, lb, lx, ly);
        vh = d2{hx, hy};
        if (!JFAST) vl = d2{lx, ly}; else vl = d2{ly, lx};
      }
      if (MUL) { vh = acc_hi[rp] * (alpha * vh); vl = acc_lo[rp] * (alpha_lo * vl); }
      else if (ACC2) {
        const d2 (&bh)[2] = (&acc_hi == &accX_hi) ? acc2X_hi : acc2Y_hi; const d2 (&bl)[2] = (&acc_hi == &accX_hi) ? acc2X_lo : acc2Y_lo;
        vh = (acc_hi[rp] + bh[rp]) + alpha * vh; vl = (acc_lo[rp] + bl[rp]) + alpha_lo * vl;
      }
      else if (ACC) { vh = acc_hi[rp] + alpha * vh; vl = acc_lo[rp] + alpha_lo * vl; }
      else if (!SG) { vh = alpha * vh; vl = alpha_lo * vl; }
      if (JFAST) { if (fold[rp]) vh = d2{vh.x, vl.y}; }
      if constexpr (PUSH) {
        typedef d2 __attribute__((address_space(1))) *gd2w;
        const u32 o = tl / tpo, q = (tl - o * tpo) * G::NT + (ng * G::NSUB + sub) * 16 + l16e;
        const bool cv = q < qmax;
        const unsigned long long of = (unsigned long long)(o + p.gfield0);
        const unsigned long long ah = (cv && o_hi[rp] != INVALID) ? pb_hi[rp] + (of * pl_hi[rp] + q) * 8ull : psink;
        const unsigned long long al = (cv && o_lo[rp] != INVALID) ? pb_lo[rp] + (of * pl_lo[rp] + q) * 8ull : psink;
        *(gd2w)ah = vh;
        *(gd2w)al = vl;
      } else {
        st16(r_out, o_hi[rp] + t0v, vh);
        st16(r_out, o_lo[rp] + t0v, vl);
      }
    }
  };

  auto run = [&](auto GRPB_) {
    constexpr bool GRPB = decltype(GRPB_)::value;
    constexpr int G_ISSUE = GRPB ? 0 : KS / 8, G_PARK = GRPB ? KS / 4 : 3 * KS / 8;
    {
      const u32 nx = tile + t_step;
      if constexpr (!ONEBUF) acc_issue(tile, true, 0, accX_hi, accX_lo);
      issue_loads(nx, nx < t_hi, 0, rjA, rmA);
#pragma unroll
      for (int q = 0; q < 4; q++) st16(r_out, INVALID, d2{0.0, 0.0});
      if constexpr (ONEBUF) acc_issue(tile, true, 0, accX_hi, accX_lo);
    }
    lds_barrier();
    STAMP3_MARK(st_loop);
    int cur = 0;
    auto tile_body = [&](auto FIRST_) {
      constexpr bool FIRST = decltype(FIRST_)::value;
      const u32 nxt = tile + t_step, nxt2 = nxt + t_step;
      const bool v1 = nxt < t_hi, v2 = nxt2 < t_hi;
      const double *sE = smem + cur * (2 * G::LDS_ELEMS), *sO = sE + G::LDS_ELEMS;
      v4d ce, co;
      chain(sE, sO, 0, G_ISSUE, G_PARK, ce, co,
            [&] { if constexpr (!ONEBUF) acc_issue(tile, true, 1, accY_hi, accY_lo); issue_loads(nxt, v1, 1, rjB, rmB); },
            [&] { park_chunk(cur ^ 1, 0, rjA, rmA); },
            [&](int g) { if constexpr (FIRST) { if (g + FA < KS / 2) frag_pair(g + FA); } });
      STAMP3(0);
      epilogue(tile, 0, ce, co, accX_hi, accX_lo);
      if constexpr (ONEBUF) acc_issue(tile, true, 1, accX_hi, accX_lo);
      STAMP3(1);
      chain(sE, sO, 1, G_ISSUE, G_PARK, ce, co,
            [&] { if constexpr (!ONEBUF) acc_issue(nxt, v1, 0, accX_hi, accX_lo); issue_loads(nxt2, v2, 0, rjA, rmA); },
            [&] { park_chunk(cur ^ 1, 1, rjB, rmB); }, [](int) {});
      STAMP3(2);
      if constexpr (ONEBUF) { epilogue(tile, 1, ce, co, accX_hi, accX_lo); acc_issue(nxt, v1, 0, accX_hi, accX_lo); }
      else epilogue(tile, 1, ce, co, accY_hi, accY_lo);
      STAMP3(3);
      lds_barrier();
      STAMP3(4);
      cur ^= 1;
    };
    tile_body(std::true_type{});
    tile += t_step;
    STAMP3_MARK(st_first);
#pragma unroll 1
    for (; tile < t_hi; tile += t_step) tile_body(std::false_type{});
  };
  if (w >= 4) run(std::true_type{}); else run(std::false_type{});
#ifdef CHEB_STAMPS
  {
    unsigned long long st_end; STAMP3_MARK(st_end);
    if (lane == 0 && p.in4) {
      unsigned long long *dbg = (unsigned long long *)p.in4 + ((size_t)BID * 8 + w) * 16;
      dbg[0] = st_seg[0]; dbg[1] = st_seg[1]; dbg[2] = st_seg[2]; dbg[3] = st_seg[3]; dbg[4] = st_seg[4];
      dbg[5] = st_loop - st_begin; dbg[6] = st_end - st_begin; dbg[7] = __builtin_amdgcn_s_memrealtime() - rt_begin;
      dbg[8] = st_wait - st_begin; dbg[9] = st_park - st_begin; dbg[10] = st_first ? st_first - st_begin : 0; dbg[11] = st_begin; dbg[12] = st_end;
    }
  }
#endif
}

template <int KS, bool JFAST, int MODE, int RAW = 0, int INM = 0, int SG = 0>
__global__ __launch_bounds__(512) void cheb_sweep_vec4_kernel(const SweepParams p) {
  __shared__ double smem[TileGeom<KS, JFAST>::LDS_DOUBLES];
  vec4_body<KS, JFAST, MODE, RAW, INM, 0, SG>(p, smem, blockIdx.x, gridDim.x);
}

template <int KS, bool PUSH>
__global__ __launch_bounds__(512) void cheb_sweep_vec4_gather_kernel(const SweepParams p, const GatherSrc g) {
  __shared__ double smem[TileGeom<KS, false>::LDS_DOUBLES];
  vec4_body<KS, false, 0, 0, 0, PUSH ? 2 : 1>(p, smem, blockIdx.x, gridDim.x, &g);
}

constexpr int MULTI_MAX = 9;
struct MultiParams { int njobs; unsigned bstart[MULTI_MAX + 1]; SweepParams job[MULTI_MAX]; };

template <int KS, bool SUM3 = false>
__global__ __launch_bounds__(512, (KS <= 8 ? 4 : 2)) void cheb_sweep_multi_kernel(const MultiParams mp) {
  constexpr int LDS = TileGeom<KS, true>::LDS_DOUBLES > TileGeom<KS, false>::LDS_DOUBLES ? TileGeom<KS, true>::LDS_DOUBLES : TileGeom<KS, false>::LDS_DOUBLES;
  __shared__ double smem[LDS];
  int j = 0;
  while (j + 1 < mp.njobs && blockIdx.x >= mp.bstart[j + 1]) j++;
  const SweepParams &p = mp.job[j];
  const u32 bid = blockIdx.x - mp.bstart[j], nblk = mp.bstart[j + 1] - mp.bstart[j];
  if (p.inner < 16) {
    if constexpr (KS >= 16) vec4_body<KS, true, 0>(p, smem, bid, nblk); else vec1_body<KS, true, SUM3, false>(p, smem, bid, nblk);
  } else {
    if constexpr (KS >= 16) vec4_body<KS, false, 0>(p, smem, bid, nblk); else vec1_body<KS, false, SUM3, false>(p, smem, bid, nblk);
  }
}

template <int KS, bool PUSH>
__global__ __launch_bounds__(512) void cheb_sweep_multi_gather_kernel(const MultiParams mp, const GatherSrc g, const unsigned gmask) {
  static_assert(KS >= 16, "the gather loader is part of the long-line kernel");
  constexpr int LDS = TileGeom<KS, true>::LDS_DOUBLES > TileGeom<KS, false>::LDS_DOUBLES ? TileGeom<KS, true>::LDS_DOUBLES : TileGeom<KS, false>::LDS_DOUBLES;
  __shared__ double smem[LDS];
  int j = 0;
  while (j + 1 < mp.njobs && blockIdx.x >= mp.bstart[j + 1]) j++;
  const SweepParams &p = mp.job[j];
  const u32 bid = blockIdx.x - mp.bstart[j], nblk = mp.bstart[j + 1] - mp.bstart[j];
  if ((gmask >> j) & 1u) vec4_body<KS, false, 0, 0, 0, PUSH ? 2 : 1>(p, smem, bid, nblk, &g);
  else if (p.inner < 16) vec4_body<KS, true, 0>(p, smem, bid, nblk);
  else vec4_body<KS, false, 0>(p, smem, bid, nblk);
}

template <int KS, bool JFAST>
static hipError_t launch_v4(const SweepParams &p, unsigned grid, hipStream_t stream) {
  if (p.in_mode == IN_MUL) {
    if (p.raw != 1 || p.out_mode != OUT_STORE) return hipErrorInvalidValue;
    hipLaunchKernelGGL((cheb_sweep_vec4_kernel<KS, JFAST, 0, 1, 1>), dim3(grid), dim3(512), 0, stream, p);
  }
  else if (p.out_mode == OUT_MUL) {
    if (p.raw != 1) return hipErrorInvalidValue;
    hipLaunchKernelGGL((cheb_sweep_vec4_kernel<KS, JFAST, 2, 1>), dim3(grid), dim3(512), 0, stream, p);
  }
  else if (p.out_mode == OUT_ACC2) {
    if (p.raw) return hipErrorInvalidValue;
    hipLaunchKernelGGL((cheb_sweep_vec4_kernel<KS, JFAST, 3>), dim3(grid), dim3(512), 0, stream, p);
  }
  else if (p.out_mode == OUT_ACC) hipLaunchKernelGGL((cheb_sweep_vec4_kernel<KS, JFAST, 1>), dim3(grid), dim3(512), 0, stream, p);
  else if (p.raw == 1) hipLaunchKernelGGL((cheb_sweep_vec4_kernel<KS, JFAST, 0, 1>), dim3(grid), dim3(512), 0, stream, p);
  else if (p.raw == 2) hipLaunchKernelGGL((cheb_sweep_vec4_kernel<KS, JFAST, 0, 2>), dim3(grid), dim3(512), 0, stream, p);
  else if (p.alpha == -1.0 && p.sym && !opt(OPT_SWEEP_ALPHA_MULTIPLY)) hipLaunchKernelGGL((cheb_sweep_vec4_kernel<KS, JFAST, 0, 0, 0, 1>), dim3(grid), dim3(512), 0, stream, p);
  else hipLaunchKernelGGL((cheb_sweep_vec4_kernel<KS, JFAST, 0>), dim3(grid), dim3(512), 0, stream, p);
  sweep_note_launch();
  return hipGetLastError();
}

template <int KS, bool JFAST>
static int prepare_v(SweepParams &p) {
  constexpr int NT = TileGeom<KS, JFAST>::NT;
  const bool custom = p.qmax != 0 || p.in_os != 0;
  if (JFAST) {
    if (!p.in_os) p.in_os = (unsigned)p.P;
    if (!p.acc_os) p.acc_os = (unsigned)p.P;
    if (!p.out_os) p.out_os = (unsigned)p.P;
    p.in_rs = p.acc_rs = p.out_rs = 1; p.nouter = p.ncols; p.qmax = 1;
    p.ntiles = (p.ncols + NT - 1) / NT;
  } else {
    if (!p.qmax) { p.qmax = p.inner; p.nouter = p.ncols / p.inner; }
    if (!p.in_os) { p.in_os = (unsigned)p.P * p.inner; p.in_rs = p.inner; }
    if (!p.acc_os) { p.acc_os = (unsigned)p.P * p.inner; p.acc_rs = p.inner; }
    if (!p.out_os) { p.out_os = (unsigned)p.P * p.inner; p.out_rs = p.inner; }
    p.ntiles = p.nouter * ((p.qmax + NT - 1) / NT);
  }
  if constexpr (KS >= 16) {
    if (!p.sink) return 0;
    const unsigned long long P_ = (unsigned long long)p.P;
    auto span = [&](unsigned os, unsigned rs) -> unsigned long long {
      if (JFAST) return ((unsigned long long)(p.ncols - 1) * os + P_) * 8ull;
      return ((unsigned long long)(p.nouter - 1) * os + (p.qmax - 1) + (P_ - 1) * rs + 1) * 8ull;
    };
    unsigned long long bi = span(p.in_os, p.in_rs);
    const unsigned long long ba = span(p.acc_os, p.acc_rs), bo = span(p.out_os, p.out_rs);
    if (p.in_fblocks) {
      const unsigned units = JFAST ? p.ncols : p.nouter;
      if (units % p.in_fblocks || (JFAST && p.in_fblocks % NT) || p.out_mode != OUT_STORE || p.raw) return 0;
      bi += (unsigned long long)(units / p.in_fblocks - 1) * p.in_fskip * 8ull;
      p.in_fblocks_inv = (unsigned)((0x100000000ull + p.in_fblocks - 1) / p.in_fblocks);
      if ((unsigned long long)(JFAST ? p.ncols + NT : p.nouter) * p.in_fblocks >= 0x100000000ull) return 0;
    }
    if (!(bi < 0x38000000ull && ba < 0x38000000ull && bo < 0x38000000ull)) return 0;
    p.in_bytes = (unsigned)bi; p.acc_bytes = (unsigned)ba; p.out_bytes = (unsigned)bo;
    return 4;
  }
  return custom ? 0 : 1;
}

template <int KS> constexpr int wgs_per_cu() { return KS <= 8 ? 2 : 1; }

template <int KS, bool JFAST>
static hipError_t launch_v(const SweepParams &p0, hipStream_t stream) {
  SweepParams p = p0;
  const int gen = prepare_v<KS, JFAST>(p);
  if (gen == 0) return hipErrorInvalidValue;
  hipError_t cu_err; int ncu = sweep_num_cus(&cu_err);
  if (cu_err != hipSuccess) return cu_err;
  ncu *= wgs_per_cu<KS>();
  const unsigned grid = p.ntiles < (unsigned)ncu ? p.ntiles : (unsigned)ncu;
  if (grid == 0) return hipSuccess;
  if constexpr (KS >= 16) return launch_v4<KS, JFAST>(p, grid, stream);
  else {
    if (p.raw && p.out_mode != OUT_STORE && !(p.out_mode == OUT_MUL && p.raw == 1)) return hipErrorInvalidValue;
    if (p.out_mode == OUT_MUL && p.raw != 1) return hipErrorInvalidValue;
    if (p.in_mode == IN_MUL) return hipErrorInvalidValue;
    if (p.out_mode == OUT_STORE) hipLaunchKernelGGL((cheb_sweep_vec_kernel<KS, JFAST, false>), dim3(grid), dim3(512), 0, stream, p);
    else hipLaunchKernelGGL((cheb_sweep_vec_kernel<KS, JFAST, true>), dim3(grid), dim3(512), 0, stream, p);
    sweep_note_launch();
    return hipGetLastError();
  }
}

template <int KS>
static bool prepare_ok_t(SweepParams p, bool jfast) { return (jfast ? prepare_v<KS, true>(p) : prepare_v<KS, false>(p)) != 0; }

bool sweep_vec_eligible(const DiffMat &m, const SweepParams &p0) {
  const SweepParams &p = p0;
  if (p.in_mode == IN_SUM3) {
    auto al16 = [](const void *q) { return q && ((size_t)q & 15) == 0; };
    if (m.KS > 8 || p.out_mode != OUT_STORE || p.raw || p.in_fblocks || p.qmax || p.in_os || !al16(p.in1) || !al16(p.in2)) return false;
  } else
  if (p.in_mode == IN_MUL) {
    if (m.KS < 16 || p.raw != 1 || p.out_mode != OUT_STORE || p.in_fblocks || p.qmax || p.in_os || !p.in1 || ((size_t)p.in1 & 15)) return false;
  } else
  if (p.out_mode == OUT_ACC2) {
    if (p.in_mode != IN_PLAIN || p.raw || p.in_fblocks || !p.acc || !p.acc2 || ((size_t)p.acc2 & 15)) return false;
  } else
  if (p.in_mode != IN_PLAIN || (p.out_mode != OUT_STORE && p.out_mode != OUT_ACC && !(p.out_mode == OUT_MUL && p.raw == 1))) return false;
  const bool jfast = p.inner < 16;
  if (p.in_fblocks && (m.KS < 16 || (p.in_fskip & 1))) return false;
  if (p.qmax != 0 || p.in_os != 0) {
    if (m.KS < 16) return false;
    const unsigned all = p.qmax | p.in_os | p.in_rs | p.acc_os | p.acc_rs | p.out_os | p.out_rs;
    if (jfast ? ((p.in_os | p.acc_os | p.out_os) & 1) : (all & 1)) return false;
  }
  if (jfast && (p.inner != 1 || (m.P & 1))) return false;
  if (!jfast && (p.inner & 1)) return false;
  auto al = [](const void *q) { return ((size_t)q & 15) == 0; };
  if (!al(p.in0) || !al(p.out) || ((p.out_mode == OUT_ACC || p.out_mode == OUT_MUL || p.out_mode == OUT_ACC2) && (!p.acc || !al(p.acc)))) return false;
  SweepParams q = p0;
  q.P = m.P; q.H = m.H; q.sink = m.sink;
  switch (m.KS) {
    case 4: return prepare_ok_t<4>(q, jfast);
    case 8: return prepare_ok_t<8>(q, jfast);
    case 16: return prepare_ok_t<16>(q, jfast);
    case 32: return prepare_ok_t<32>(q, jfast);
    default: return false;
  }
}

bool sweep_vec_raw_eligible(const DiffMat &m, const SweepParams &p0) {
  if ((p0.out_mode != OUT_STORE && !(p0.out_mode == OUT_MUL && p0.raw == 1)) || opt(OPT_NO_RAW_TRANSFORMS) || opt(OPT_GENERAL_KERNELS)) return false;
  return sweep_vec_eligible(m, p0);
}

hipError_t sweep_vec_launch(const DiffMat &m, SweepParams p, hipStream_t stream) {
  if (p.in_mode == IN_SUM3) return hipErrorInvalidValue;
  const bool jfast = p.inner < 16;
  switch (m.KS) {
    case 4: return jfast ? launch_v<4, true>(p, stream) : launch_v<4, false>(p, stream);
    case 8: return jfast ? launch_v<8, true>(p, stream) : launch_v<8, false>(p, stream);
    case 16: return jfast ? launch_v<16, true>(p, stream) : launch_v<16, false>(p, stream);
    case 32: return jfast ? launch_v<32, true>(p, stream) : launch_v<32, false>(p, stream);
    default: return hipErrorInvalidValue;
  }
}

template <int KS>
static hipError_t launch_gather_t(SweepParams p, const GatherSrc &g, hipStream_t stream, bool *done) {
  const int gen = prepare_v<KS, false>(p);
  if (gen != 4) return hipSuccess;
  hipError_t cu_err; const int ncu = sweep_num_cus(&cu_err);
  if (cu_err != hipSuccess) return cu_err;
  const unsigned grid = p.ntiles < (unsigned)ncu ? p.ntiles : (unsigned)ncu;
  *done = true;
  if (grid == 0) return hipSuccess;
  if (g.push) hipLaunchKernelGGL((cheb_sweep_vec4_gather_kernel<KS, true>), dim3(grid), dim3(512), 0, stream, p, g);
  else hipLaunchKernelGGL((cheb_sweep_vec4_gather_kernel<KS, false>), dim3(grid), dim3(512), 0, stream, p, g);
  sweep_note_launch();
  return hipGetLastError();
}

static bool gather_ok(const DiffMat &m, SweepParams &p, const GatherSrc &g) {
  if (m.KS < 16 || p.inner < 16 || (p.inner & 1) || p.in_mode != IN_PLAIN || p.out_mode != OUT_STORE || p.raw || p.in_fblocks || p.qmax || p.in_os) return false;
  if (g.G < 1 || g.G > GATHER_MAX || (g.rowlen & 1) || (g.col0 & 1) || (size_t)g.col0 + p.inner > g.rowlen) return false;
  for (int s = 0; s < g.G; s++) if (!g.p[s] || ((size_t)g.p[s] & 15) || (g.lq[s] & 1) || g.pmax[s] < 1 || g.s0[s + 1] < g.s0[s]) return false;
  if (g.push) { for (int s = 0; s < g.G; s++) if (!g.dp[s] || ((size_t)g.dp[s] & 15)) return false; if (!p.out) return false; }
  if (g.s0[0] != 0 || g.s0[g.G] != m.P) return false;
  p.in0 = g.p[0];
  return sweep_vec_eligible(m, p);
}
hipError_t sweep_vec_launch_gather(const DiffMat &m, SweepParams p, const GatherSrc &g, hipStream_t stream, bool *done) {
  *done = false;
  if (!gather_ok(m, p, g)) return hipSuccess;
  switch (m.KS) {
    case 16: return launch_gather_t<16>(p, g, stream, done);
    case 32: return launch_gather_t<32>(p, g, stream, done);
    default: return hipSuccess;
  }
}

template <int KS>
static hipError_t launch_multi_t(int n, SweepParams *jobs, hipStream_t stream, bool *done, const GatherSrc *g = nullptr, unsigned gmask = 0) {
  if (g && KS < 16) { *done = false; return hipSuccess; }
  for (int j = 0; j < n; j++) if (jobs[j].raw || jobs[j].in_mode == IN_MUL) { *done = false; return hipSuccess; }
  bool sum3 = jobs[0].in_mode == IN_SUM3;
  for (int j = 1; j < n; j++) if ((jobs[j].in_mode == IN_SUM3) != sum3) { *done = false; return hipSuccess; }
  if (sum3 && KS > 8) { *done = false; return hipSuccess; }
  MultiParams mp = {};
  mp.njobs = n;
  hipError_t cu_err; int ncu = sweep_num_cus(&cu_err);
  if (cu_err != hipSuccess) return cu_err;
  ncu *= wgs_per_cu<KS>();
  unsigned long long total = 0;
  for (int j = 0; j < n; j++) {
    SweepParams &p = jobs[j];
    const bool jfast = p.inner < 16;
    const int gen = jfast ? prepare_v<KS, true>(p) : prepare_v<KS, false>(p);
    if (gen == 0) return hipSuccess;
    total += p.ntiles;
  }
  const int split = opt(OPT_EQUAL_SHARES) ? 0 : 1;
  unsigned gs[MULTI_MAX];
  for (int j = 0; j < n; j++) {
    const unsigned nt = jobs[j].ntiles;
    gs[j] = ((nt < (unsigned)ncu ? nt : (unsigned)ncu) + 7u) & ~7u;
  }
  if (split && total > (unsigned long long)ncu && ncu % 8 == 0 && ncu >= 8 * n) {
    const unsigned units = (unsigned)ncu / 8u;
    unsigned u[MULTI_MAX], used = 0;
    unsigned long long rem[MULTI_MAX];
    for (int j = 0; j < n; j++) {
      const unsigned long long x = (unsigned long long)units * jobs[j].ntiles;
      u[j] = (unsigned)(x / total); rem[j] = x % total;
      if (u[j] == 0 && jobs[j].ntiles) { u[j] = 1; rem[j] = 0; }
      used += u[j];
    }
    while (used < units) {
      int best = 0;
      for (int j = 1; j < n; j++) if (rem[j] > rem[best]) best = j;
      u[best]++; rem[best] = 0; used++;
    }
    if (used == units) {
      for (int j = 0; j < n; j++) if (8u * u[j] < gs[j]) gs[j] = 8u * u[j];
      auto walk = [&](unsigned nt, unsigned g_) -> unsigned {
        if (g_ == 0) return nt ? 0xffffffffu : 0u;
        if (g_ % 8 == 0) { const unsigned per = (nt + 7) / 8, w8 = g_ / 8; return (per + w8 - 1) / w8; }
        return (nt + g_ - 1) / g_;
      };
      unsigned span_al = 0;
      for (int j = 0; j < n; j++) { const unsigned w_ = walk(jobs[j].ntiles, gs[j]); span_al = w_ > span_al ? w_ : span_al; }
      unsigned g1[MULTI_MAX], used1 = 0; unsigned long long rem1[MULTI_MAX];
      for (int j = 0; j < n; j++) {
        const unsigned long long x = (unsigned long long)ncu * jobs[j].ntiles;
        g1[j] = (unsigned)(x / total); rem1[j] = x % total;
        if (g1[j] == 0 && jobs[j].ntiles) { g1[j] = 1; rem1[j] = 0; }
        used1 += g1[j];
      }
      while (used1 < (unsigned)ncu) { int best = 0; for (int j = 1; j < n; j++) if (rem1[j] > rem1[best]) best = j; g1[best]++; rem1[best] = 0; used1++; }
      if (used1 == (unsigned)ncu) {
        unsigned span_1 = 0;
        for (int j = 0; j < n; j++) { const unsigned w_ = walk(jobs[j].ntiles, g1[j]); span_1 = w_ > span_1 ? w_ : span_1; }
        if (span_1 < span_al) for (int j = 0; j < n; j++) gs[j] = g1[j] < jobs[j].ntiles ? g1[j] : jobs[j].ntiles;
      }
    }
  }
  unsigned b = 0;
  for (int j = 0; j < n; j++) { mp.bstart[j] = b; b += gs[j]; mp.job[j] = jobs[j]; }
  mp.bstart[n] = b;
#ifdef CHEB_STAMPS
  if (::chebhip_stamp_buf()) {
    const int set = ::chebhip_stamp_next() & 1;
    for (int j = 0; j < n; j++) mp.job[j].in4 = ::chebhip_stamp_buf() + (size_t)3 * (256 * 8 * 16) + (size_t)(set * 9 + j) * (512 * 8 * 16);
  }
#endif
  if (b == 0) { *done = true; return hipSuccess; }
  if constexpr (KS <= 8) {
    if (sum3) hipLaunchKernelGGL((cheb_sweep_multi_kernel<KS, true>), dim3(b), dim3(512), 0, stream, mp);
    else hipLaunchKernelGGL((cheb_sweep_multi_kernel<KS>), dim3(b), dim3(512), 0, stream, mp);
  } else {
    if (g && g->push) hipLaunchKernelGGL((cheb_sweep_multi_gather_kernel<KS, true>), dim3(b), dim3(512), 0, stream, mp, *g, gmask);
    else if (g) hipLaunchKernelGGL((cheb_sweep_multi_gather_kernel<KS, false>), dim3(b), dim3(512), 0, stream, mp, *g, gmask);
    else hipLaunchKernelGGL((cheb_sweep_multi_kernel<KS>), dim3(b), dim3(512), 0, stream, mp);
  }
  sweep_note_launch();
  *done = true;
  return hipGetLastError();
}

hipError_t sweep_vec_launch_multi(int n, const DiffMat *const *m, SweepParams *jobs, hipStream_t stream, bool *done) {
  *done = false;
  if (n < 1 || n > MULTI_MAX) return hipSuccess;
  for (int j = 0; j < n; j++) {
    if (m[j]->KS != m[0]->KS || jobs[j].out_mode != OUT_STORE || !sweep_vec_eligible(*m[j], jobs[j])) return hipSuccess;
  }
  switch (m[0]->KS) {
    case 4: return launch_multi_t<4>(n, jobs, stream, done);
    case 8: return launch_multi_t<8>(n, jobs, stream, done);
    case 16: return launch_multi_t<16>(n, jobs, stream, done);
    case 32: return launch_multi_t<32>(n, jobs, stream, done);
    default: return hipSuccess;
  }
}

hipError_t sweep_vec_launch_multi_gather(int n, const DiffMat *const *m, SweepParams *jobs, unsigned gmask, const GatherSrc &g, hipStream_t stream, bool *done) {
  *done = false;
  if (n < 2 || n > MULTI_MAX || gmask == 0 || (gmask >> n) != 0) return hipSuccess;
  for (int j = 0; j < n; j++) {
    if (m[j]->KS != m[0]->KS || jobs[j].out_mode != OUT_STORE) return hipSuccess;
    if (((gmask >> j) & 1u) ? !gather_ok(*m[j], jobs[j], g) : !sweep_vec_eligible(*m[j], jobs[j])) return hipSuccess;
  }
  switch (m[0]->KS) {
    case 16: return launch_multi_t<16>(n, jobs, stream, done, &g, gmask);
    case 32: return launch_multi_t<32>(n, jobs, stream, done, &g, gmask);
    default: return hipSuccess;
  }
}

}
```

spectral-petsc_amd/csrc/tile.h:

```cpp
#pragma once
#include <hip/hip_runtime.h>

namespace chebhip {

typedef double v4d __attribute__((ext_vector_type(4)));
typedef double d2 __attribute__((ext_vector_type(2)));
typedef unsigned u32;
typedef unsigned v4u __attribute__((ext_vector_type(4)));
typedef unsigned v2u __attribute__((ext_vector_type(2)));

template <int KS, bool JFAST, int LB = 16>
struct TileGeom {
  static constexpr int MTP = KS / 4;
  static constexpr int NG = 8 / MTP;
  static constexpr int HP = 4 * KS;
  static constexpr int NSUB = (KS >= 16) ? 2 : 1;
  static constexpr int NT = 16 * NG * NSUB;
  static constexpr int LDJ = HP + 1;
  static constexpr int LDS_ELEMS = JFAST ? NT * LDJ : HP * NT;
  static constexpr int PER = LB / 8;
  static constexpr int ITEMS = HP * NT / PER / 512;
  static constexpr int CH = ITEMS / NSUB;
  static constexpr int LD_W = (JFAST ? HP : NT) / PER;
  static constexpr int QSTEP = 512 / LD_W;
  static constexpr int LDS_QSTEP = JFAST ? QSTEP * LDJ : QSTEP * NT;
  static constexpr int KSTR = JFAST ? 4 : 4 * NT;
  static constexpr int NFL = (KS == 32) ? (JFAST ? 7 : 8) : 0;
  static constexpr int KR = KS - NFL;
  static constexpr int LDS_DOUBLES = 4 * LDS_ELEMS + 8 * NFL * 64;
  static_assert(LB == 8 || LB == 16, "8- or 16-byte loader slots");

  static __device__ __forceinline__ int at(int i, int n) { return JFAST ? n * LDJ + i : i * NT + (n ^ ((i & 1) << 4)); }
  static __device__ __forceinline__ int frag(int nb, int l16, int kq) { return JFAST ? (nb + l16) * LDJ + kq : kq * NT + ((nb + l16) ^ ((kq & 1) << 4)); }
};

__device__ __forceinline__ void lds_barrier() { asm volatile("s_waitcnt lgkmcnt(0)\n\ts_barrier" ::: "memory"); }

struct TileWalk {
  u32 bid, nxcd, t_lo, t_hi, t_step;
  __device__ __forceinline__ u32 rank() const { return bid / nxcd; }
  __device__ __forceinline__ u32 first() const { return t_lo + bid / nxcd; }
};
__device__ __forceinline__ TileWalk tile_walk(u32 bid, u32 nblk, u32 ntiles) {
  const u32 nxcd = (nblk % 8 == 0) ? 8u : 1u;
  const u32 t_per = (ntiles + nxcd - 1) / nxcd;
  const u32 t_lo = (bid % nxcd) * t_per;
  const u32 t_hi = (t_lo + t_per < ntiles) ? t_lo + t_per : ntiles;
  return TileWalk{bid, nxcd, t_lo, t_hi, nblk / nxcd};
}

template <int KS, bool JFAST, int KSTR, class AE, class AO, class HOOK>
__device__ __forceinline__ void mfma_chain(const double *fE, const double *fO, v4d &ce, v4d &co, AE &&ae, AO &&ao, HOOK &&hook) {
  double fb[2][4];
  fb[0][0] = fE[0]; fb[0][1] = fE[KSTR]; fb[0][2] = fO[0]; fb[0][3] = fO[KSTR];
#pragma unroll
  for (int g = 0; g < KS / 2; g++) {
    const int cb = g & 1, nbuf = cb ^ 1;
    if (g + 1 < KS / 2) {
      fb[nbuf][0] = fE[(2 * g + 2) * KSTR]; fb[nbuf][1] = fE[(2 * g + 3) * KSTR];
      fb[nbuf][2] = fO[(2 * g + 2) * KSTR]; fb[nbuf][3] = fO[(2 * g + 3) * KSTR];
    }
    __builtin_amdgcn_sched_barrier(0);
    hook(g);
    if (!JFAST) {
      ce = __builtin_amdgcn_mfma_f64_16x16x4f64(ae(2 * g), fb[cb][0], ce, 0, 0, 0);
      co = __builtin_amdgcn_mfma_f64_16x16x4f64(ao(2 * g), fb[cb][2], co, 0, 0, 0);
      ce = __builtin_amdgcn_mfma_f64_16x16x4f64(ae(2 * g + 1), fb[cb][1], ce, 0, 0, 0);
      co = __builtin_amdgcn_mfma_f64_16x16x4f64(ao(2 * g + 1), fb[cb][3], co, 0, 0, 0);
    } else {
      ce = __builtin_amdgcn_mfma_f64_16x16x4f64(fb[cb][0], ae(2 * g), ce, 0, 0, 0);
      co = __builtin_amdgcn_mfma_f64_16x16x4f64(fb[cb][2], ao(2 * g), co, 0, 0, 0);
      ce = __builtin_amdgcn_mfma_f64_16x16x4f64(fb[cb][1], ae(2 * g + 1), ce, 0, 0, 0);
      co = __builtin_amdgcn_mfma_f64_16x16x4f64(fb[cb][3], ao(2 * g + 1), co, 0, 0, 0);
    }
  }
}

template <int KR>
__device__ __forceinline__ double frag_odd(int k, const double *ao, const double *aoL) { return (k < KR) ? ao[(k < KR) ? k : 0] : aoL[(k - KR) * 64]; }

__device__ __forceinline__ double swap1(double v) {
  int lo = __double2loint(v), hi = __double2hiint(v);
  lo = __builtin_amdgcn_update_dpp(lo, lo, 0xB1, 0xF, 0xF, false);
  hi = __builtin_amdgcn_update_dpp(hi, hi, 0xB1, 0xF, 0xF, false);
  return __hiloint2double(hi, lo);
}
__device__ __forceinline__ double bc_even(double v) {
  int lo = __double2loint(v), hi = __double2hiint(v);
  lo = __builtin_amdgcn_update_dpp(0, lo, 0xA0, 0xF, 0xF, true); hi = __builtin_amdgcn_update_dpp(0, hi, 0xA0, 0xF, 0xF, true);
  return __hiloint2double(hi, lo);
}
__device__ __forceinline__ double bc_odd(double v) {
  int lo = __double2loint(v), hi = __double2hiint(v);
  lo = __builtin_amdgcn_update_dpp(0, lo, 0xF5, 0xF, 0xF, true); hi = __builtin_amdgcn_update_dpp(0, hi, 0xF5, 0xF, 0xF, true);
  return __hiloint2double(hi, lo);
}

constexpr unsigned long long PAIR_EVEN = 0x5555555555555555ull, PAIR_ODD = 0xAAAAAAAAAAAAAAAAull;
__device__ __forceinline__ void xpair(double a, double b, double &x, double &y) {
  const int al = __double2loint(a), ah = __double2hiint(a), bl = __double2loint(b), bh = __double2hiint(b);
  int xl, xh, yl, yh;
  asm("s_mov_b64 vcc, %8\n\t"
      "s_nop 1\n\t"
      "v_cndmask_b32_dpp %0, %6, %4, vcc quad_perm:[0,0,2,2] row_mask:0xf bank_mask:0xf\n\t"
      "v_cndmask_b32_dpp %1, %7, %5, vcc quad_perm:[0,0,2,2] row_mask:0xf bank_mask:0xf\n\t"
      "s_mov_b64 vcc, %9\n\t"
      "v_cndmask_b32_dpp %2, %4, %6, vcc quad_perm:[1,1,3,3] row_mask:0xf bank_mask:0xf\n\t"
      "v_cndmask_b32_dpp %3, %5, %7, vcc quad_perm:[1,1,3,3] row_mask:0xf bank_mask:0xf"
      : "=&v"(xl), "=&v"(xh), "=&v"(yl), "=&v"(yh) : "v"(al), "v"(ah), "v"(bl), "v"(bh), "s"(PAIR_EVEN), "s"(PAIR_ODD) : "vcc");
  x = __hiloint2double(xh, xl); y = __hiloint2double(yh, yl);
}

__device__ __forceinline__ d2 ld16(__amdgpu_buffer_rsrc_t r, u32 off) { return __builtin_bit_cast(d2, __builtin_amdgcn_raw_buffer_load_b128(r, (int)off, 0, 0)); }
__device__ __forceinline__ void st16(__amdgpu_buffer_rsrc_t r, u32 off, d2 v) { __builtin_amdgcn_raw_buffer_store_b128(__builtin_bit_cast(v4u, v), r, (int)off, 0, 0); }
__device__ __forceinline__ double ld8(__amdgpu_buffer_rsrc_t r, u32 off) { return __builtin_bit_cast(double, __builtin_amdgcn_raw_buffer_load_b64(r, (int)off, 0, 0)); }
__device__ __forceinline__ void st8(__amdgpu_buffer_rsrc_t r, u32 off, double v) { __builtin_amdgcn_raw_buffer_store_b64(__builtin_bit_cast(v2u, v), r, (int)off, 0, 0); }

}
```

Before: 4165 matvecs/s.

## Rebase buffer resources per tile to lift the 896MB array size cap

The vec4 sweep kernel now builds a buffer resource per tile, based at the tile origin with a remaining-length bound, instead of one whole-array resource with byte offsets. This lets arrays exceed the old ~0.9 GB limit that forced a fallback to slower sweep paths. Invalid loads are now masked through a zero-size resource, and partial-column stores use an exec mask. It also adds a separate launch counter for vec kernels. In exchange, every tile pays extra scalar work to build resources, and the inline exec-mask assembly is fragile.

```diff
diff --git a/include/chebhip.h b/include/chebhip.h
--- a/include/chebhip.h
+++ b/include/chebhip.h
@@ -367,6 +367,7 @@
 const char *chebhip_option_name(int index);
 
 long chebhip_launch_count(void);
+long chebhip_vec_launch_count(void);
 
 enum {
   CHEBHIP_STAGE_CHEB_APPLY = 0, CHEBHIP_STAGE_ELL_MULT, CHEBHIP_STAGE_ELL_FUNCTION, CHEBHIP_STAGE_STOKES_MULT,
diff --git a/spectral-petsc_amd/__init__.py b/spectral-petsc_amd/__init__.py
--- a/spectral-petsc_amd/__init__.py
+++ b/spectral-petsc_amd/__init__.py
@@ -7,7 +7,7 @@
 INCLUDE_DIR = os.path.join(os.path.dirname(_HERE), "include")
 
 ABI_SYMBOLS = [
-    "chebhip_last_error", "chebhip_version", "chebhip_arch", "chebhip_launch_count",
+    "chebhip_last_error", "chebhip_version", "chebhip_arch", "chebhip_launch_count", "chebhip_vec_launch_count",
     "chebhip_set_option", "chebhip_get_option", "chebhip_option_name",
     "cheb_plan_create", "cheb_apply", "cheb_apply_host", "cheb_plan_destroy", "cheb_plan_size",
     "cheb_plan_create_trimmed", "cheb_apply_lap1d", "cheb_slab_pack", "cheb_slab_unpack_add",
@@ -100,6 +100,7 @@
         L.chebhip_last_error.restype = C.c_char_p
         L.chebhip_arch.restype = C.c_char_p
         L.chebhip_launch_count.restype = C.c_long
+        L.chebhip_vec_launch_count.restype = C.c_long
         L.chebhip_set_option.argtypes = [C.c_char_p, C.c_int]
         L.chebhip_get_option.argtypes = [C.c_char_p, C.POINTER(C.c_int)]
         L.chebhip_option_name.argtypes = [C.c_int]
diff --git a/spectral-petsc_amd/csrc/chebhip.hip b/spectral-petsc_amd/csrc/chebhip.hip
--- a/spectral-petsc_amd/csrc/chebhip.hip
+++ b/spectral-petsc_amd/csrc/chebhip.hip
@@ -28,6 +28,7 @@
 extern "C" int chebhip_version(void) { return 100; }
 extern "C" const char *chebhip_arch(void) { return "gfx950"; }
 extern "C" long chebhip_launch_count(void) { return sweep_launch_count(); }
+extern "C" long chebhip_vec_launch_count(void) { return sweep_vec_launch_count(); }
 
 extern "C" int chebhip_set_option(const char *name, int value) {
   if (!name) return chebhip_fail(CHEBHIP_ERR_ARG, "NULL option name");
diff --git a/spectral-petsc_amd/csrc/sweep.h b/spectral-petsc_amd/csrc/sweep.h
--- a/spectral-petsc_amd/csrc/sweep.h
+++ b/spectral-petsc_amd/csrc/sweep.h
@@ -54,7 +54,7 @@
   double *gout;
   unsigned nouter, qmax;
   unsigned in_os, in_rs, acc_os, acc_rs, out_os, out_rs;
-  unsigned in_bytes, acc_bytes, out_bytes;
+  unsigned in_len, acc_len, out_len;
   unsigned in_fblocks, in_fskip;
   unsigned in_fblocks_inv;
   unsigned gfield0;
@@ -150,6 +150,7 @@
 hipError_t sweep_launch_multi_try(int n, const DiffMat *const *m, const SweepParams *p, hipStream_t stream, bool *done);
 
 long sweep_launch_count();
+long sweep_vec_launch_count();
 }
 struct cheb_plan;
 struct stokes_op;
diff --git a/spectral-petsc_amd/csrc/sweep_vec.hip b/spectral-petsc_amd/csrc/sweep_vec.hip
--- a/spectral-petsc_amd/csrc/sweep_vec.hip
+++ b/spectral-petsc_amd/csrc/sweep_vec.hip
@@ -1,5 +1,6 @@
 #include "sweep.h"
 #include "tile.h"
+#include <atomic>
 #include <cstdlib>
 #include <type_traits>
 
@@ -7,6 +8,10 @@
 int chebhip_stamp_next();
 
 namespace chebhip {
+
+static std::atomic<long> g_vec_launches{0};
+long sweep_vec_launch_count() { return g_vec_launches.load(); }
+static void note_vec_launch() { g_vec_launches.fetch_add(1); sweep_note_launch(); }
 
 template <bool ALIGNED16>
 __device__ __forceinline__ void lds_put2(double *dst, double __attribute__((ext_vector_type(2))) v) {
@@ -322,7 +327,7 @@
   static_assert(!MUL || RAW == 1, "OUT_MUL exists for the raw forward transform only");
   static_assert(SG == 0 || (MODE == 0 && RAW == 0 && INM == 0 && GATH == 0), "the sign-only store exists for the plain STORE launch");
   using G = TileGeom<KS, JFAST>;
-  constexpr u32 INVALID = 0x80000000u, T_INVALID = 0x40000000u;
+  constexpr u32 INVALID = 0x80000000u;
   static_assert(KS >= 16 && G::CH >= 1, "v4 needs two sub-tiles per tile");
 
 #ifdef CHEB_STAMPS
@@ -337,11 +342,8 @@
   const int nn = p.P - 1, H = p.H;
   const u32 qmax = p.qmax;
 
-  const __amdgpu_buffer_rsrc_t r_in = __builtin_amdgcn_make_buffer_rsrc((void *)p.in0, 0, p.in_bytes, 0x00020000);
-  const __amdgpu_buffer_rsrc_t r_in1 = __builtin_amdgcn_make_buffer_rsrc((void *)(INM ? p.in1 : p.in0), 0, INM ? p.in_bytes : 0u, 0x00020000);
-  const __amdgpu_buffer_rsrc_t r_acc = __builtin_amdgcn_make_buffer_rsrc((void *)(ACC ? p.acc : p.in0), 0, ACC ? p.acc_bytes : 0u, 0x00020000);
-  const __amdgpu_buffer_rsrc_t r_acc2 = __builtin_amdgcn_make_buffer_rsrc((void *)(ACC2 ? p.acc2 : p.in0), 0, ACC2 ? p.acc_bytes : 0u, 0x00020000);
-  const __amdgpu_buffer_rsrc_t r_out = __builtin_amdgcn_make_buffer_rsrc((void *)p.out, 0, p.out_bytes, 0x00020000);
+
+  const __amdgpu_buffer_rsrc_t r_whole = __builtin_amdgcn_make_buffer_rsrc((void *)p.out, 0, (GATH == 1) ? p.out_len * 8u : 0u, 0x00020000);
 
   double ae[KS], ao[G::KR > 0 ? G::KR : 1];
   double *aoL = smem + 4 * G::LDS_ELEMS + (w * G::NFL) * 64 + lane;
@@ -354,20 +356,23 @@
   const int ld_lds0 = JFAST ? ld_b * G::LDJ + 2 * ld_a : ld_b * G::NT + ((2 * ld_a) ^ ((ld_b & 1) << 4));
   const u32 in_os8 = p.in_os * 8u, in_rs8 = p.in_rs * 8u;
   const u32 lj = JFAST ? (u32)ld_b * in_os8 + (u32)(2 * ld_a) * 8u : (u32)(2 * ld_a) * 8u + (u32)ld_b * in_rs8;
-  const u32 lm = JFAST ? (u32)ld_b * in_os8 + (u32)(nn - 2 * ld_a - 1) * 8u : (u32)(2 * ld_a) * 8u + (u32)(nn - ld_b) * in_rs8;
-  const u32 slot8 = JFAST ? (u32)G::QSTEP * in_os8 : (u32)G::QSTEP * in_rs8;
-  auto tile_off = [&](u32 tl, bool valid, u32 os8) -> u32 {
-    if (JFAST) return valid ? tl * G::NT * os8 : T_INVALID;
+  const u32 lm = JFAST ? (u32)ld_b * in_os8 + (u32)(nn - 2 * ld_a - 1) * 8u : (u32)(2 * ld_a) * 8u + (u32)(nn - ld_b - (G::ITEMS - 1) * G::QSTEP) * in_rs8;
+  const u32 slot = JFAST ? (u32)G::QSTEP * p.in_os : (u32)G::QSTEP * p.in_rs;
+  static_assert(G::CH == 2 && G::ITEMS == 4, "two chunks of two loader slots");
+  auto slot_of = [](int chunk, int s) -> int { return (JFAST || GATH) ? chunk * G::CH + s : (s == 0 ? chunk : G::ITEMS - 1 - chunk); };
+  auto tile_org = [&](u32 tl, u32 os) -> u32 {
+    if (JFAST) return tl * G::NT * os;
     const u32 o = tl / tpo, q0 = (tl - o * tpo) * G::NT;
-    return valid ? o * os8 + q0 * 8u : T_INVALID;
-  };
-
-  const u32 fb = p.in_fblocks, fskip8 = p.in_fskip * 8u;
-  auto in_tile_off = [&](u32 tl) -> u32 {
-    u32 off = tile_off(tl, true, in_os8);
-    if (fb) off += __umulhi(JFAST ? tl * G::NT : tl / tpo, p.in_fblocks_inv) * fskip8;
-    return off;
-  };
+    return o * os + q0;
+  };
+  const u32 fb = p.in_fblocks;
+  auto in_tile_org = [&](u32 tl) -> u32 {
+    u32 org = tile_org(tl, p.in_os);
+    if (fb) org += __umulhi(JFAST ? tl * G::NT : tl / tpo, p.in_fblocks_inv) * p.in_fskip;
+    return org;
+  };
+  const u32 ngs = (G::NG == 1) ? 0u : (u32)__builtin_amdgcn_readfirstlane(ng);
+  auto sub_org = [&](int sub, u32 os) -> u32 { return (ngs * G::NSUB + (u32)sub) * 16u * (JFAST ? os : 1u); };
 
   typedef const d2 __attribute__((address_space(1))) *gd2p;
   unsigned long long gb_j[GATH ? G::ITEMS : 1], gb_m[GATH ? G::ITEMS : 1];
@@ -424,27 +429,27 @@
       u32 qq = q0 + 2u * (u32)ld_a; if (qq > qmax - 2u) qq = qmax - 2u;
 #pragma unroll
       for (int s = 0; s < G::CH; s++) {
-        const int sg = chunk * G::CH + s;
+        const int sg = slot_of(chunk, s);
         rj[s] = *(gd2p)(gb_j[sg] + ((unsigned long long)(o + gf0) * glq_j[sg] + qq) * 8ull);
         rm[s] = *(gd2p)(gb_m[sg] + ((unsigned long long)(o + gf0) * glq_m[sg] + qq) * 8ull);
       }
       return;
     }
-    const u32 t0 = in_tile_off(tl);
+    const u32 org = in_tile_org(tl);
     if constexpr (INM != 0) {
       d2 (&ej)[ECH] = (&rj == &rjA) ? ejA : ejB; d2 (&em)[ECH] = (&rj == &rjA) ? emA : emB;
 #pragma unroll
       for (int s = 0; s < G::CH; s++) {
-        const u32 so = (u32)(chunk * G::CH + s) * slot8;
-        ej[s] = ld16(r_in1, lj + (valid ? t0 + so : T_INVALID));
-        em[s] = ld16(r_in1, lm + (valid ? (JFAST ? t0 + so : t0 - so) : T_INVALID));
+        const int sg = slot_of(chunk, s), sm = JFAST ? sg : G::ITEMS - 1 - sg;
+        ej[s] = ld16(rsrc_at(p.in1, p.in_len, org + (u32)sg * slot, valid), lj);
+        em[s] = ld16(rsrc_at(p.in1, p.in_len, org + (u32)sm * slot, valid), lm);
       }
     }
 #pragma unroll
     for (int s = 0; s < G::CH; s++) {
-      const u32 so = (u32)(chunk * G::CH + s) * slot8;
-      rj[s] = ld16(r_in, lj + (valid ? t0 + so : T_INVALID));
-      rm[s] = ld16(r_in, lm + (valid ? (JFAST ? t0 + so : t0 - so) : T_INVALID));
+      const int sg = slot_of(chunk, s), sm = JFAST ? sg : G::ITEMS - 1 - sg;
+      rj[s] = ld16(rsrc_at(p.in0, p.in_len, org + (u32)sg * slot, valid), lj);
+      rm[s] = ld16(rsrc_at(p.in0, p.in_len, org + (u32)sm * slot, valid), lm);
     }
   };
   const bool oddP = (p.P & 1) != 0;
@@ -452,7 +457,7 @@
     double *dE = smem + buf * (2 * G::LDS_ELEMS), *dO = dE + G::LDS_ELEMS;
 #pragma unroll
     for (int s = 0; s < G::CH; s++) {
-      const int idx = ld_lds0 + (chunk * G::CH + s) * G::LDS_QSTEP;
+      const int idx = ld_lds0 + slot_of(chunk, s) * G::LDS_QSTEP;
       d2 e, o;
       d2 xj = rj[s], xm = rm[s];
       if constexpr (INM != 0) {
@@ -465,7 +470,7 @@
       } else if (!JFAST) {
         e = xj + xm;
         o = xj - xm;
-        if (oddP) { asm volatile("" ::: "memory"); const bool mid = 2 * (ld_b + (chunk * G::CH + s) * G::QSTEP) == nn; if (mid) e = xj; }
+        if (oddP) { asm volatile("" ::: "memory"); const bool mid = 2 * (ld_b + slot_of(chunk, s) * G::QSTEP) == nn; if (mid) e = xj; }
       } else {
         e = d2{xj.x + xm.y, xj.y + xm.x};
         o = d2{xj.x - xm.y, xj.y - xm.x};
@@ -499,20 +504,19 @@
       c_lo[rp] = (u32)(4 * r + kq) * (p.acc_os * 8u) + (u32)(ok ? nn - ie - 1 : 0) * 8u;
     }
   }
-  const u32 out_os8 = p.out_os * 8u, acc_os8 = p.acc_os * 8u;
-  const u32 sub8_out = JFAST ? 16u * out_os8 : 16u * 8u, sub8_acc = JFAST ? 16u * acc_os8 : 16u * 8u;
-  const u32 ng8_out = (u32)ng * G::NSUB * sub8_out, ng8_acc = (u32)ng * G::NSUB * sub8_acc;
   const double alpha = p.alpha, alpha_lo = (p.sym || RAW == 1) ? p.alpha : -p.alpha;
 
   auto acc_issue = [&](u32 tl, bool valid, int sub, d2 (&ah)[2], d2 (&al)[2]) {
     if (!ACC) return;
-    const u32 t0 = tile_off(tl, valid, acc_os8) + ng8_acc + (u32)sub * sub8_acc;
-#pragma unroll
-    for (int rp = 0; rp < 2; rp++) { ah[rp] = ld16(r_acc, c_hi[rp] + t0); al[rp] = ld16(r_acc, c_lo[rp] + t0); }
+    const u32 org = tile_org(tl, p.acc_os) + sub_org(sub, p.acc_os);
+    const __amdgpu_buffer_rsrc_t r_acc = rsrc_at(p.acc, p.acc_len, org, valid);
+#pragma unroll
+    for (int rp = 0; rp < 2; rp++) { ah[rp] = ld16(r_acc, c_hi[rp]); al[rp] = ld16(r_acc, c_lo[rp]); }
     if constexpr (ACC2) {
       d2 (&bh)[2] = (&ah == &accX_hi) ? acc2X_hi : acc2Y_hi; d2 (&bl)[2] = (&ah == &accX_hi) ? acc2X_lo : acc2Y_lo;
-#pragma unroll
-      for (int rp = 0; rp < 2; rp++) { bh[rp] = ld16(r_acc2, c_hi[rp] + t0); bl[rp] = ld16(r_acc2, c_lo[rp] + t0); }
+      const __amdgpu_buffer_rsrc_t r_acc2 = rsrc_at(p.acc2, p.acc_len, org, valid);
+#pragma unroll
+      for (int rp = 0; rp < 2; rp++) { bh[rp] = ld16(r_acc2, c_hi[rp]); bl[rp] = ld16(r_acc2, c_lo[rp]); }
     }
   };
 
@@ -561,11 +565,22 @@
                                    [&](int g) { grp_fn(g); if (g == g_issue) issue_fn(); if (g == g_park) park_fn(); });
   };
   auto epilogue = [&](u32 tl, int sub, const v4d &ce, const v4d &co, const d2 (&acc_hi)[2], const d2 (&acc_lo)[2]) {
-    u32 t0 = tile_off(tl, true, out_os8) + ng8_out + (u32)sub * sub8_out;
-    u32 t0v = t0;
-    if (!JFAST) {
-      const u32 o = tl / tpo, q = (tl - o * tpo) * G::NT + (ng * G::NSUB + sub) * 16 + l16e;
-      t0v = (q < qmax) ? t0 : T_INVALID;
+    const __amdgpu_buffer_rsrc_t r_out = (GATH == 1) ? r_whole : rsrc_at(p.out, p.out_len, tile_org(tl, p.out_os) + sub_org(sub, p.out_os), true);
+    unsigned long long cols = ~0ull;
+    u32 g_t0v = 0;
+    if constexpr (GATH == 1) {
+      const u32 o = tl / tpo, q0 = (tl - o * tpo) * G::NT + sub_org(sub, 1u);
+      g_t0v = (q0 + (u32)l16e < qmax) ? (o * p.out_os + q0) * 8u : 0x40000000u;
+    }
+    if (!JFAST && !GATH) {
+      const u32 o = tl / tpo;
+      const u32 left = qmax - (tl - o * tpo) * G::NT, c0 = sub_org(sub, 1u);
+      u32 c0x = c0;
+      asm("" : "+s"(c0x));
+      u32 k = (left > c0x ? left : c0x) - c0;
+      k = k < 16u ? k : 16u;
+      const u32 m16 = (1u << k) - 1u, m32 = m16 | (m16 << 16);
+      cols = (unsigned long long)m32 | ((unsigned long long)m32 << 32);
     }
     double hi[4], lo[4];
 #pragma unroll
@@ -606,9 +621,19 @@
         const unsigned long long al = (cv && o_lo[rp] != INVALID) ? pb_lo[rp] + (of * pl_lo[rp] + q) * 8ull : psink;
         *(gd2w)ah = vh;
         *(gd2w)al = vl;
+      } else if (GATH == 1) {
+        st16(r_out, o_hi[rp] + g_t0v, vh);
+        st16(r_out, o_lo[rp] + g_t0v, vl);
+      } else if (JFAST) {
+        st16(r_out, o_hi[rp], vh);
+        st16(r_out, o_lo[rp], vl);
       } else {
-        st16(r_out, o_hi[rp] + t0v, vh);
-        st16(r_out, o_lo[rp] + t0v, vl);
+        __builtin_amdgcn_sched_barrier(0);
+        asm volatile("s_mov_b64 exec, %0" :: "s"(cols) : "memory");
+        st16(r_out, o_hi[rp], vh);
+        st16(r_out, o_lo[rp], vl);
+        asm volatile("s_mov_b64 exec, -1" ::: "memory");
+        __builtin_amdgcn_sched_barrier(0);
       }
     }
   };
@@ -621,7 +646,7 @@
       if constexpr (!ONEBUF) acc_issue(tile, true, 0, accX_hi, accX_lo);
       issue_loads(nx, nx < t_hi, 0, rjA, rmA);
 #pragma unroll
-      for (int q = 0; q < 4; q++) st16(r_out, INVALID, d2{0.0, 0.0});
+      for (int q = 0; q < 4; q++) st16((GATH == 1) ? r_whole : rsrc_at(p.out, p.out_len, 0u, false), INVALID, d2{0.0, 0.0});
       if constexpr (ONEBUF) acc_issue(tile, true, 0, accX_hi, accX_lo);
     }
     lds_barrier();
@@ -735,7 +760,7 @@
   else if (p.raw == 2) hipLaunchKernelGGL((cheb_sweep_vec4_kernel<KS, JFAST, 0, 2>), dim3(grid), dim3(512), 0, stream, p);
   else if (p.alpha == -1.0 && p.sym && !opt(OPT_SWEEP_ALPHA_MULTIPLY)) hipLaunchKernelGGL((cheb_sweep_vec4_kernel<KS, JFAST, 0, 0, 0, 1>), dim3(grid), dim3(512), 0, stream, p);
   else hipLaunchKernelGGL((cheb_sweep_vec4_kernel<KS, JFAST, 0>), dim3(grid), dim3(512), 0, stream, p);
-  sweep_note_launch();
+  note_vec_launch();
   return hipGetLastError();
 }
 
@@ -772,12 +797,20 @@
       p.in_fblocks_inv = (unsigned)((0x100000000ull + p.in_fblocks - 1) / p.in_fblocks);
       if ((unsigned long long)(JFAST ? p.ncols + NT : p.nouter) * p.in_fblocks >= 0x100000000ull) return 0;
     }
-    if (!(bi < 0x38000000ull && ba < 0x38000000ull && bo < 0x38000000ull)) return 0;
-    p.in_bytes = (unsigned)bi; p.acc_bytes = (unsigned)ba; p.out_bytes = (unsigned)bo;
+    auto window = [&](unsigned os, unsigned rs) -> unsigned long long {
+      constexpr unsigned long long HP2 = 2ull * TileGeom<KS, JFAST>::HP;
+      return (JFAST ? (unsigned long long)NT * os + HP2 : HP2 * rs + NT) * 8ull;
+    };
+    const unsigned long long wi = window(p.in_os, p.in_rs), wa = window(p.acc_os, p.acc_rs), wo = window(p.out_os, p.out_rs);
+    if (!(wi < 0x40000000ull && wa < 0x40000000ull && wo < 0x40000000ull)) return 0;
+    if (!(bi + wi < 0x800000000ull && ba + wa < 0x800000000ull && bo + wo < 0x800000000ull)) return 0;
+    p.in_len = (unsigned)(bi / 8ull); p.acc_len = (unsigned)(ba / 8ull); p.out_len = (unsigned)(bo / 8ull);
     return 4;
   }
   return custom ? 0 : 1;
 }
+
+static bool gather_out_ok(const SweepParams &p) { return (unsigned long long)p.out_len * 8ull < 0x38000000ull; }
 
 template <int KS> constexpr int wgs_per_cu() { return KS <= 8 ? 2 : 1; }
 
@@ -798,7 +831,7 @@
     if (p.in_mode == IN_MUL) return hipErrorInvalidValue;
     if (p.out_mode == OUT_STORE) hipLaunchKernelGGL((cheb_sweep_vec_kernel<KS, JFAST, false>), dim3(grid), dim3(512), 0, stream, p);
     else hipLaunchKernelGGL((cheb_sweep_vec_kernel<KS, JFAST, true>), dim3(grid), dim3(512), 0, stream, p);
-    sweep_note_launch();
+    note_vec_launch();
     return hipGetLastError();
   }
 }
@@ -861,7 +894,7 @@
 template <int KS>
 static hipError_t launch_gather_t(SweepParams p, const GatherSrc &g, hipStream_t stream, bool *done) {
   const int gen = prepare_v<KS, false>(p);
-  if (gen != 4) return hipSuccess;
+  if (gen != 4 || !gather_out_ok(p)) return hipSuccess;
   hipError_t cu_err; const int ncu = sweep_num_cus(&cu_err);
   if (cu_err != hipSuccess) return cu_err;
   const unsigned grid = p.ntiles < (unsigned)ncu ? p.ntiles : (unsigned)ncu;
@@ -869,7 +902,7 @@
   if (grid == 0) return hipSuccess;
   if (g.push) hipLaunchKernelGGL((cheb_sweep_vec4_gather_kernel<KS, true>), dim3(grid), dim3(512), 0, stream, p, g);
   else hipLaunchKernelGGL((cheb_sweep_vec4_gather_kernel<KS, false>), dim3(grid), dim3(512), 0, stream, p, g);
-  sweep_note_launch();
+  note_vec_launch();
   return hipGetLastError();
 }
 
@@ -909,7 +942,7 @@
     SweepParams &p = jobs[j];
     const bool jfast = p.inner < 16;
     const int gen = jfast ? prepare_v<KS, true>(p) : prepare_v<KS, false>(p);
-    if (gen == 0) return hipSuccess;
+    if (gen == 0 || (g && ((gmask >> j) & 1u) && !gather_out_ok(p))) return hipSuccess;
     total += p.ntiles;
   }
   const int split = opt(OPT_EQUAL_SHARES) ? 0 : 1;
@@ -975,7 +1008,7 @@
     else if (g) hipLaunchKernelGGL((cheb_sweep_multi_gather_kernel<KS, false>), dim3(b), dim3(512), 0, stream, mp, *g, gmask);
     else hipLaunchKernelGGL((cheb_sweep_multi_kernel<KS>), dim3(b), dim3(512), 0, stream, mp);
   }
-  sweep_note_launch();
+  note_vec_launch();
   *done = true;
   return hipGetLastError();
 }
diff --git a/spectral-petsc_amd/csrc/tile.h b/spectral-petsc_amd/csrc/tile.h
--- a/spectral-petsc_amd/csrc/tile.h
+++ b/spectral-petsc_amd/csrc/tile.h
@@ -111,6 +111,15 @@
   x = __hiloint2double(xh, xl); y = __hiloint2double(yh, yl);
 }
 
+constexpr u32 RSRC_MAX_RECORDS = 0x80000000u;
+__device__ __forceinline__ __amdgpu_buffer_rsrc_t rsrc_at(const double *a, u32 len, u32 org, bool valid) {
+  u32 orgx = org;
+  asm("" : "+s"(orgx));
+  u32 rem = (len > orgx ? len : orgx) - org;
+  rem = rem < RSRC_MAX_RECORDS / 8u ? rem : RSRC_MAX_RECORDS / 8u;
+  return __builtin_amdgcn_make_buffer_rsrc((void *)(a + org), 0, valid ? rem * 8u : 0u, 0x00020000);
+}
+
 __device__ __forceinline__ d2 ld16(__amdgpu_buffer_rsrc_t r, u32 off) { return __builtin_bit_cast(d2, __builtin_amdgcn_raw_buffer_load_b128(r, (int)off, 0, 0)); }
 __device__ __forceinline__ void st16(__amdgpu_buffer_rsrc_t r, u32 off, d2 v) { __builtin_amdgcn_raw_buffer_store_b128(__builtin_bit_cast(v4u, v), r, (int)off, 0, 0); }
 __device__ __forceinline__ double ld8(__amdgpu_buffer_rsrc_t r, u32 off) { return __builtin_bit_cast(double, __builtin_amdgcn_raw_buffer_load_b64(r, (int)off, 0, 0)); }
```

Result: faster. 4232 matvecs/s, median of 6 (+1.6%).
